# MaxHalford/sorobn

Measured on AMD Instinct MI355X. Metric: exact posterior queries/sec on 100-node 4-state grid BN, higher is better.
Workload: dtype f64

## Files before the change

__graft_entry__.py:

```python
import os
import subprocess
import sys

ROOT = os.path.dirname(os.path.abspath(__file__))
CSRC = os.path.join(ROOT, "sorobn_amd", "csrc")
LIB = os.path.join(ROOT, "sorobn_amd", "libmibn.so")
SOURCES = [os.path.join(CSRC, f) for f in ("planner.cpp", "engine.hip")]
DEPS = SOURCES + [os.path.join(CSRC, f) for f in ("planner.h", "plan_policy.h", "device_mem.h", "emit_core.h", "order_search.h", "ve_kernel.hip.h", "sweep_kernel.hip.h", "tiny_kernel.hip.h", "gibbs_kernel.hip.h", "sampler_plan.h",
                                              "sample_kernel.hip.h", "count_kernel.hip.h", "wave_prims.h", "wave_plan.h", "wave_plan_kernel.hip.h", "elim_kernel.hip.h", "draw_kernel.hip.h", "expect_kernel.hip.h", "score_kernel.hip.h", "citest_kernel.hip.h", "likelihood_kernel.hip.h", "bp_plan.h", "bp_kernel.hip.h", "count_weighted_kernel.hip.h")] + \
    [os.path.join(ROOT, "include", "mibn.h")]


def _stale(target, deps):
    if not os.path.exists(target):
        return True
    t = os.path.getmtime(target)
    return any(os.path.getmtime(d) > t for d in deps)


def build(force: bool = False) -> None:
    hipcc = os.environ.get("HIPCC", "/opt/rocm/bin/hipcc")
    if force or _stale(LIB, DEPS):
        cmd = [hipcc, "--offload-arch=gfx950", "-O3", "-mpopcnt", "-std=c++17", "-fPIC", "-shared",
               "-Wno-unused-value", "-Wno-unused-result", "-I", os.path.join(ROOT, "include"),
               "-o", LIB, *SOURCES, "-lpthread", "-ldl"]
        print("[build]", " ".join(cmd), flush=True)
        subprocess.check_call(cmd)
    subprocess.check_call(["make", "-C", os.path.join(ROOT, "oracle"), "-s"])
    if ROOT not in sys.path:
        sys.path.insert(0, ROOT)
    import sorobn_amd
    from sorobn_amd import _capi
    L = _capi.lib()
    missing = [s for s in _capi.SYMBOLS if not hasattr(L, s)]
    assert not missing, f"libmibn.so lacks {missing}"
    print("[build] ok:", L.mibn_version().decode(), flush=True)


def smoke() -> None:
    for p in (ROOT, os.path.join(ROOT, "tests")):
        if p not in sys.path:
            sys.path.insert(0, p)
    import numpy as np

    import netspec
    import sorobn_amd
    from oracle.oracle import OracleNet

    nets = netspec.load(os.path.join(ROOT, "tests", "golden", "examples.json"))
    alarm = next(n for n in nets if n["spec"]["name"] == "alarm")["spec"]
    checks = [(alarm, ("Burglary",), {"Mary calls": True, "John calls": True}),
              (netspec.grid_spec(4, 4, 4), ("000",), {"015": 0}),
              (netspec.grid_spec(6, 6, 4), ("035", "007"), {"000": 0, "020": 3})]
    for spec, q, ev in checks:
        bn = netspec.build(spec, sorobn_amd.BayesNet).use_device(0)
        ans = bn.query(*q, event=ev)
        names, labels, vals = OracleNet(spec).query(q, ev)
        assert list(ans.index.names) == names, (ans.index.names, names)
        assert [k if isinstance(k, tuple) else (k,) for k in ans.index.tolist()] == labels
        err = float(np.max(np.abs(ans.to_numpy() - vals)))
        assert err <= 1e-9, err
        print(f"[smoke] {spec['name']} P({', '.join(q)}) = {ans.to_numpy().tolist()} max|err| vs oracle {err:.2e}",
              flush=True)
    import golden_util as gu
    entry = gu.load("grid10x10.json")
    bn = netspec.build(gu.grid_spec_from_recipe(entry), sorobn_amd.BayesNet).use_device(0)
    reqs = [r for r in entry["requests"] if r["query"] == ["099"] and r["event"] == [["000", 0]]] + entry["requests"][:6]
    answers = bn.query_many([(tuple(r["query"]), {k: v for k, v in r["event"]}) for r in reqs])
    worst = 0.0
    for r, ans in zip(reqs, answers):
        name, inames, rows, vals, multi = gu.expected(r)
        assert ans.name == name and list(ans.index.names) == inames
        gu.assert_rows_equal(ans.index.tolist(), rows, ctx=str(r["query"]))
        worst = max(worst, float(np.max(np.abs(ans.to_numpy() - vals))))
    assert worst <= gu.TOL, worst
    st = bn.backend.engine.stats()
    print(f"[smoke] 10x10 K=4 grid: {len(reqs)} requests vs the reference's own answers, max|err| {worst:.2e}; "
          f"{st['alg_bytes'] / 1e6:.0f} MB algorithmic in {st['kernel_ms']:.2f} ms of kernels", flush=True)
    bn.backend.engine.set_option("second_on_device", 1)
    bn.backend.engine.set_option("gpu_emit", 2)
    again = bn.query_many([(tuple(r["query"]), {k: v for k, v in r["event"]}) for r in reqs])
    assert all(np.array_equal(a.to_numpy(), b.to_numpy()) for a, b in zip(answers, again))
    planned = [k for k in bn.backend.engine.kernel_stats() if k["name"] == "order_kernel+emit_kernel"]
    assert planned and planned[0]["items"] == len(reqs), planned
    print(f"[smoke] device planner: {len(reqs)} programs word for word the host's, posteriors bit for bit", flush=True)
    print("[smoke] ok", flush=True)


if __name__ == "__main__":
    build(force="--force" in sys.argv)
    if "--smoke" in sys.argv:
# ... 2 lines not shown
```

sorobn_amd/csrc/engine.hip:

```cpp
#include <hip/hip_runtime.h>
#include <dlfcn.h>
#include <rccl/rccl.h>

#include <algorithm>
#include <atomic>
#include <chrono>
#include <condition_variable>
#include <cstdio>
#include <cstdlib>
#include <cstring>
#include <limits>
#include <memory>
#include <mutex>
#include <numeric>
#include <string>
#include <thread>
#include <vector>

#include "../../include/mibn.h"
#include "device_mem.h"
#include "gibbs_kernel.hip.h"
#include "bp_kernel.hip.h"
#include "sample_kernel.hip.h"
#include "count_kernel.hip.h"
#include "count_weighted_kernel.hip.h"
#include "score_kernel.hip.h"
#include "citest_kernel.hip.h"
#include "planner.h"
#include "plan_policy.h"
#include "tiny_kernel.hip.h"
#include "sweep_kernel.hip.h"
#include "ve_kernel.hip.h"
#include "draw_kernel.hip.h"
#include "elim_kernel.hip.h"
#include "expect_kernel.hip.h"
#include "likelihood_kernel.hip.h"
#include "wave_plan_kernel.hip.h"

using namespace mibn;

namespace {
double now_ms() {
    return std::chrono::duration<double, std::milli>(std::chrono::steady_clock::now().time_since_epoch()).count();
}
}

struct OrderArgs {
    OrderNet net;
    const int64_t *q_off, *e_off;
    const int32_t *q_vars, *e_vars;
    int64_t B;
    uint32_t flags;
    uint8_t *orders;
    int32_t *order_len;
    OrderScratch *scratch;
    uint32_t *zero;
    const int32_t *perm;
    int32_t lanes;
};

#ifndef MIBN_ORDER_WAVES_PER_EU
#define MIBN_ORDER_WAVES_PER_EU 4
#endif
#ifndef MIBN_EMIT_WAVES_PER_EU
#define MIBN_EMIT_WAVES_PER_EU 4
#endif
#ifndef MIBN_PLAN_WG
#define MIBN_PLAN_WG 1024
#endif
__global__ __launch_bounds__(MIBN_PLAN_WG, MIBN_ORDER_WAVES_PER_EU) void order_kernel(const OrderArgs A) {
    if (A.zero && blockIdx.x == 0 && threadIdx.x == 0) *A.zero = 0;
    const int lane = (int)(threadIdx.x & 63), wave = (int)(threadIdx.x >> 6), waves = (int)(blockDim.x >> 6);
    if (lane >= A.lanes) return;
    const int64_t pos = ((int64_t)blockIdx.x * waves + wave) * A.lanes + lane;
    if (pos >= A.B) return;
    const int64_t b = A.perm ? A.perm[pos] : pos;
    OrderScratch &S = A.scratch[pos];
    const int64_t q0 = A.q_off[b], e0 = A.e_off[b];
    order_search(A.net, S, (int)(A.q_off[b + 1] - q0), A.q_vars + q0, (int)(A.e_off[b + 1] - e0), A.e_vars + e0,
                 (A.flags & MIBN_Q_NOPRUNE) != 0);
    uint8_t *out = A.orders + b * 128;
    for (int i = 0; i < S.n_best; ++i) out[i] = S.best[i];
    A.order_len[b] = S.n_best;
}

struct EmitArgs {
    EmitNet net;
    const int64_t *q_off, *e_off, *out_off;
    const int32_t *q_vars, *e_vars, *e_codes;
    const char *skip;
    const uint8_t *orders;
    const int32_t *order_len;
    int64_t B;
    uint32_t flags;
    uint32_t *prog;
    uint32_t prog_stride;
    EmitMeta *meta;
    Tag *tags;
    uint32_t *tag_cursor;
    uint32_t tag_cap;
    char *scratch;
    size_t scratch_stride;
    const int32_t *perm;
    int32_t lanes;
};

#if defined(MIBN_EMIT_PROF)
__device__ unsigned long long g_emit_prof[12];
#endif

__global__ __launch_bounds__(MIBN_PLAN_WG, MIBN_EMIT_WAVES_PER_EU) void emit_kernel(const EmitArgs A) {
    const int lane = (int)(threadIdx.x & 63), wave = (int)(threadIdx.x >> 6), waves = (int)(blockDim.x >> 6);
    if (lane >= A.lanes) return;
    const int64_t pos = ((int64_t)blockIdx.x * waves + wave) * A.lanes + lane;
    if (pos >= A.B) return;
    const int64_t b = A.perm ? A.perm[pos] : pos;
    EmitMeta m;
    m.words = 1; m.n_tags = 0; m.tag_first = 0; m.err = 0; m.prog_first = 0; m.pad_ = 0;
    m.alg_bytes = m.alg_flops = m.n_steps = m.max_step_cells = 0;
    m.arena_cells = 0;
    uint32_t *slot = A.prog + (size_t)b * A.prog_stride;
    if (A.skip[b]) { slot[0] = 0; A.meta[b] = m; return; }
// ... 175 lines not shown
    int set_cursor = 0;
    uint64_t call_id = 0;
    struct Comm {
        Stream stream;
        void *dl = nullptr;
        ncclComm_t comm = nullptr;
        int rank = 0, world = 1;
        decltype(&ncclGetUniqueId) GetUniqueId = nullptr;
        decltype(&ncclCommInitRank) CommInitRank = nullptr;
        decltype(&ncclCommDestroy) CommDestroy = nullptr;
        decltype(&ncclCommCount) CommCount = nullptr;
        decltype(&ncclCommUserRank) CommUserRank = nullptr;
        decltype(&ncclAllGather) AllGather = nullptr;
        decltype(&ncclReduce) Reduce = nullptr;
        decltype(&ncclAllReduce) AllReduce = nullptr;
        decltype(&ncclGetErrorString) GetErrorString = nullptr;
        DevBuf<char> d_send, d_recv;
    } comm;
    std::string err;
    mibn_stats stats{}, total{};
    mibn_kernel_stat kstats[kStatSlots];
    mibn_kernel_stat ktotal[kStatSlots];
    struct Elim {
        std::vector<ProgBuf> bufs;
        BatchPlan plan;
        Schedule sched;
        std::vector<LaunchGroup> groups;
        DevBuf<uint32_t> d_prog;
        DevBuf<uint64_t> d_prog_off, d_arena_off;
        DevBuf<Item> d_items;
        DevBuf<uint32_t> d_wg_item;
        DevBuf<double> d_m, d_log_p;
        DevBuf<int32_t> d_codes;
        DevBuf<DrawItem> d_draw_items;
        DevBuf<int64_t> d_m_off;
        ChunkSeeds seeds;
        std::vector<Event> ev;
        ~Elim() { for (ProgBuf &b : bufs) b.release(); }
    } elim;
    struct Expect {
        ExpectPlan plan;
        const double *weight = nullptr;
        int64_t B = 0, n_acc = 0;
        double *acc = nullptr, *p_out = nullptr;
        DevBuf<char> d_meta;
        DevBuf<double> d_f64;
        Event ev[2];
    } ex;
    bool expect = false;
    Findings staged;
    bool has_staged = false;
    const Findings *lh = nullptr;
    struct Dataset {
        DevBuf<uint8_t> d_codes;
        int64_t n_rows = 0;
        int32_t n_cols = 0;
        std::vector<int32_t> card;
        bool live = false;
        DevBuf<uint32_t> d_weights;
        int32_t n_sets = 0;
        std::vector<int64_t> weight_sum;
    };
    std::vector<Dataset> datasets;
    struct Score {
        DevBuf<unsigned long long> d_counts;
        DevBuf<char> d_meta;
        DevBuf<double> d_f64;
        DevBuf<long long> d_i64;
        std::vector<Event> ev;
    } sc;
    int64_t score_cells = kScoreCellBudget;
    int weighted_share = 1;
    double arena_gb = 200.0;
    int mfma_kernel = 1;
    int seg_kernel = 1;
    Event epoch;
    Event lane_ev, zero_ev;
    double busy_until = 0;
    int n_streams = 1;
    int first_chunk = 1;
    int threads = 0;
    int trace = 0;
    int split_kinds = 0;
    int overlap = 1;
    int sweep_dma = 1;
    int gibbs_lds = 1;
    int bp_lds = 1;
    int64_t chunk = 32768;
};

#define HIP_TRY(h, expr)                                                                              \
    do {                                                                                              \
        hipError_t e_ = (expr);                                                                       \
        if (e_ != hipSuccess) {                                                                       \
            (h)->err = std::string(#expr) + ": " + hipGetErrorString(e_);                             \
            return MIBN_E_HIP;                                                                        \
        }                                                                                             \
    } while (0)

static int upload_order_net(mibn_ctx *h) {
    h->order_net_ok = false;
    if (h->planner_only || h->net.n_vars > 128 || h->net.n_vars < 1) return MIBN_OK;
    const Network &net = h->net;
    const size_t n = (size_t)net.n_vars, nh = net.hint_sorted.size();
    std::vector<char> buf;
    auto put = [&](const void *p, size_t bytes) {
        const size_t off = (buf.size() + 15) & ~size_t(15);
        buf.resize(off + bytes);
        if (bytes) std::memcpy(buf.data() + off, p, bytes);
        return off;
    };
    const size_t o_card = put(net.card.data(), n * 4), o_depth = put(net.depth.data(), n * 4);
    const size_t o_asc = put(net.topo_asc.data(), n * 4), o_desc = put(net.topo_desc.data(), n * 4);
    const size_t o_hint = put(net.hint_flat.data(), nh * n * 4), o_log = put(net.log2card.data(), n * 8);
    const size_t o_anc = put(net.anc2.data(), n * sizeof(B2)), o_sc = put(net.scope2.data(), n * sizeof(B2));
    const size_t o_fam = put(net.fam2.data(), n * sizeof(B2));
    HIP_TRY(h, h->d_order_net.reset(buf.size()));
    HIP_TRY(h, hipMemcpy(h->d_order_net, buf.data(), buf.size(), hipMemcpyHostToDevice));
    OrderNet &o = h->order_net_dev;
    o = net.order_view();
    char *d = h->d_order_net;
    o.card = reinterpret_cast<const int32_t *>(d + o_card);
    o.depth = reinterpret_cast<const int32_t *>(d + o_depth);
    o.topo_asc = reinterpret_cast<const int32_t *>(d + o_asc);
    o.topo_desc = reinterpret_cast<const int32_t *>(d + o_desc);
    o.hint_sorted = reinterpret_cast<const int32_t *>(d + o_hint);
    o.log2card = reinterpret_cast<const double *>(d + o_log);
    o.anc = reinterpret_cast<const B2 *>(d + o_anc);
    o.cpt_scope = reinterpret_cast<const B2 *>(d + o_sc);
    o.fam = reinterpret_cast<const B2 *>(d + o_fam);
    h->order_net_ok = true;
    return MIBN_OK;
}

static int upload_emit_net(mibn_ctx *h) {
    h->emit_net_ok = false;
    if (h->planner_only || h->net.n_vars > 128 || h->net.n_vars < 1) return MIBN_OK;
    const Network &net = h->net;
    const size_t n = (size_t)net.n_vars;
    std::vector<char> buf;
    auto put = [&](const void *p, size_t bytes) {
        const size_t off = (buf.size() + 15) & ~size_t(15);
        buf.resize(off + bytes);
        if (bytes) std::memcpy(buf.data() + off, p, bytes);
        return off;
    };
    const size_t o_card = put(net.card.data(), n * 4), o_log = put(net.log2card.data(), n * 8), o_pool = put(net.pool_off.data(), n * 8);
    const size_t o_soff = put(net.scope_off32.data(), (n + 1) * 4), o_sv = put(net.scope_flat.data(), net.scope_flat.size() * 4);
    const size_t o_ss = put(net.cstride_flat.data(), net.cstride_flat.size() * 8), o_anc = put(net.anc_flat.data(), net.anc_flat.size() * 8);
    HIP_TRY(h, h->d_emit_net.reset(buf.size()));
    HIP_TRY(h, hipMemcpy(h->d_emit_net, buf.data(), buf.size(), hipMemcpyHostToDevice));
    EmitNet &e = h->emit_net_dev;
    e = net.emit_view();
    char *d = h->d_emit_net;
    e.card = reinterpret_cast<const int32_t *>(d + o_card);
    e.log2card = reinterpret_cast<const double *>(d + o_log);
    e.pool_off = reinterpret_cast<const int64_t *>(d + o_pool);
    e.scope_off = reinterpret_cast<const int32_t *>(d + o_soff);
    e.scope_vars = reinterpret_cast<const int32_t *>(d + o_sv);
    e.scope_stride = reinterpret_cast<const int64_t *>(d + o_ss);
    e.anc = reinterpret_cast<const uint64_t *>(d + o_anc);
    h->emit_net_ok = true;
    return MIBN_OK;
}

enum : unsigned { kNeedIdle = 1, kNeedDevice = 2, kNeedNet = 4 };
static int check_state(mibn_ctx *h, unsigned need) {
    if ((need & kNeedIdle) && (h->pend[0].active || h->pend[1].active)) { h->err = "asynchronous calls in flight: collect them with mibn_wait first"; return MIBN_E_STATE; }
    if ((need & kNeedDevice) && h->planner_only) { h->err = "planner-only context: no HIP device bound (there is no CPU fallback)"; return MIBN_E_NODEVICE; }
    if ((need & kNeedNet) && !h->has_net) { h->err = "set_network first"; return MIBN_E_STATE; }
    return MIBN_OK;
}

extern "C" {

const char *mibn_version(void) { return "mibn 0.1 (gfx950)"; }

int mibn_device_count(int *count) {
    int n = 0;
    if (hipGetDeviceCount(&n) != hipSuccess) n = 0;
    if (count) *count = n;
    return MIBN_OK;
}

constexpr int kEngineSmallCells = 512;

int mibn_create_planner(mibn_t **out) {
    if (!out) return MIBN_E_ARG;
    auto *h = new mibn_ctx();
    h->net.order_effort = 1; h->net.second_above = h->pol.base_second_above;
    h->net.small_cells = kEngineSmallCells;
    h->net.minfill_above = h->pol.base_minfill;
    h->planner_only = true;
    *out = h;
    return MIBN_OK;
}

int mibn_create(int device, mibn_t **out) {
    if (!out) return MIBN_E_ARG;
    *out = nullptr;
    int n = 0;
    if (hipGetDeviceCount(&n) != hipSuccess || n <= 0) return MIBN_E_NODEVICE;
    if (device < 0 || device >= n) return MIBN_E_ARG;
    auto *h = new mibn_ctx();
    h->net.order_effort = 1; h->net.second_above = h->pol.base_second_above;
    h->net.small_cells = kEngineSmallCells;
    h->net.minfill_above = h->pol.base_minfill;
    h->device = device;
    if (hipSetDevice(device) != hipSuccess) { delete h; return MIBN_E_NODEVICE; }
    hipDeviceProp_t prop;
    if (hipGetDeviceProperties(&prop, device) != hipSuccess) { delete h; return MIBN_E_NODEVICE; }
    if (std::string(prop.gcnArchName).rfind("gfx950", 0) != 0) {
        delete h;
        return MIBN_E_NODEVICE;
    }
    h->n_cu = prop.multiProcessorCount;
    bool ok = true;
    for (Stream *q : {&h->stream, &h->stream2, &h->aux[0][0], &h->aux[0][1], &h->aux[1][0], &h->aux[1][1], &h->aux[0][2], &h->aux[1][2], &h->copy_stream})
        ok = ok && q->ensure(hipStreamNonBlocking) == hipSuccess;
    ok = ok && hipFuncSetAttribute((const void *)ve_sweep_kernel, hipFuncAttributeMaxDynamicSharedMemorySize, kSweepLdsBytes) == hipSuccess;
    ok = ok && hipFuncSetAttribute((const void *)ve_sweep_dma_kernel, hipFuncAttributeMaxDynamicSharedMemorySize, kSweepLdsBytes) == hipSuccess;
    if (!ok) { delete h; return MIBN_E_HIP; }
    *out = h;
    return MIBN_OK;
}

void mibn_destroy(mibn_t *h) {
    if (!h) return;
    if (!h->planner_only) {
        (void)hipSetDevice(h->device);
        if (h->stream) (void)hipStreamSynchronize(h->stream);
        if (h->stream2) (void)hipStreamSynchronize(h->stream2);
        (void)mibn_comm_destroy(h);
    }
    delete h;
}

const char *mibn_last_error(const mibn_t *h) { return h ? h->err.c_str() : "null handle"; }

int mibn_set_option(mibn_t *h, const char *name, double value) {
    if (!h || !name) return MIBN_E_ARG;
    std::string n(name);
    if (n == "arena_gb") h->arena_gb = value;
    else if (n == "threads") h->threads = (int)value;
    else if (n == "chunk") h->chunk = std::max<int64_t>(1, (int64_t)value);
    else if (n == "big_iters") h->net.big_iters = std::max<int64_t>(1, (int64_t)value);
    else if (n == "tile_h") h->net.tile_h = std::max(0, std::min(kTileMax, (int)value));
    else if (n == "tile_kb") h->net.tile_bytes = std::max<int64_t>(16, (int64_t)value) << 10;
    else if (n == "chunk_sets") { if (mibn_drain(h) != MIBN_OK) return MIBN_E_HIP; h->n_sets = std::max(2, std::min(kChunkSets, (int)value)); h->set_cursor = 0; }
    else if (n == "trace") h->trace = (int)value;
    else if (n == "split_kinds") h->split_kinds = value != 0;
    else if (n == "overlap") { if (mibn_drain(h) != MIBN_OK) return MIBN_E_HIP; h->overlap = value != 0; }
    else if (n == "sweep_dma") h->sweep_dma = value != 0;
    else if (n == "seg_kernel") h->seg_kernel = value != 0;
    else if (n == "gibbs_lds") h->gibbs_lds = std::max(0, std::min(2, (int)value));
    else if (n == "bp_lds") h->bp_lds = value != 0;
    else if (n == "tiny") h->tiny = value != 0;
    else if (n == "tiny_zero_copy") h->tiny_zero_copy = value != 0;
    else if (n == "mfma_kernel") h->mfma_kernel = value != 0;
    else if (n == "gpu_emit") h->gpu_emit = std::max(0, std::min(2, (int)value));
    else if (n == "wave_wgs") h->wave_wgs = std::max(0, (int)value);
    else if (n == "plan_priority") h->plan_priority = std::max(0, std::min(2, (int)value));
    else if (n == "wave_plan") h->wave_plan = value != 0;
    else if (n == "plan_waves") h->plan_waves = std::max(1, std::min(16, (int)value));
    else if (n == "plan_sort") h->plan_sort = (int)value;
    else if (n == "wave_sort") h->wave_sort = value != 0;
    else if (n == "plan_lanes") h->plan_lanes = std::max(0, std::min(64, (int)value));
    else if (n == "emit_share") { h->pol.emit_share_opt = value > 0 ? std::min(1.0, value) : -1; if (value > 0) h->pol.emit_share = h->pol.emit_share_opt; }
    else if (n == "emit_words") h->emit_words = (uint32_t)std::max(1024, std::min(1 << 20, (int)value));
    else if (n == "gpu_search") h->gpu_search = std::max(0, std::min(2, (int)value));
    else if (n == "adaptive") {
        h->pol.adaptive = value != 0;
        if (!h->pol.adaptive) {
            h->net.minfill_above = h->pol.base_minfill;
            if (h->pol.auto_emit) { h->gpu_emit = 0; h->pol.auto_emit = false; }
            if (h->pol.auto_search) { h->gpu_search = 0; h->pol.auto_search = false; }
            h->pol.adaptive_seeded = false;
        }
    }
    else if (n == "minfill_above") { h->pol.base_minfill = value; h->net.minfill_above = value; }
    else if (n == "fuse") h->net.fuse = value != 0;
    else if (n == "plan_cache") h->net.plan_cache = value != 0;
    else if (n == "chain") h->net.chain = value != 0;
    else if (n == "streams") { if (mibn_drain(h) != MIBN_OK) return MIBN_E_HIP; h->n_streams = value >= 2 ? 2 : 1; h->n_sets = 2 * h->n_streams; h->set_cursor = 0; }
    else if (n == "first_chunk") h->first_chunk = std::max(0, std::min(2, (int)value));
    else if (n == "builtin_sweeps") {
        h->net.builtin_sweeps = value != 0;
        if (h->net.n_vars > 0) {
            std::vector<int32_t> flat;
            for (const auto &hh : h->net.hints) flat.insert(flat.end(), hh.begin(), hh.end());
            h->net.set_hints((int32_t)h->net.hints.size(), flat.data());
            if (!h->planner_only) return upload_order_net(h);
        }
    }
    else if (n == "order_effort") h->net.order_effort = std::max(0, std::min(1, (int)value));
    else if (n == "second_above") { h->pol.base_second_above = value; h->net.second_above = value; }
    else if (n == "second_on_device") h->second_on_device = value != 0;
    else if (n == "order_weights") h->net.order_weights = std::max(0, std::min(64, (int)value));
    else if (n == "sweep_canon") h->net.sweep_canon = value != 0;
    else if (n == "sweep_adapt") h->net.sweep_adapt = std::max(0, (int)value);
    else if (n == "sweep_min") h->net.sweep_min = std::max(2, std::min(5, (int)value));
    else if (n == "sweep_iters") h->net.sweep_iters = std::max(1, std::min(kTileMax, (int)value));
    else if (n == "sweep") h->net.sweep = std::max(0, std::min(5, (int)value));
    else if (n == "outer") h->net.outer = value != 0;
    else if (n == "stagger") h->net.stagger = std::max(1, std::min(8, (int)value));
    else if (n == "prune") h->net.prune = value != 0;
    else if (n == "weighted_share") h->weighted_share = value != 0;
    else if (n == "score_cells") h->score_cells = std::max<int64_t>(1, std::min<int64_t>(int64_t(1) << 28, (int64_t)value));
    else if (n == "small_cells") h->net.small_cells = std::max(1, std::min(kMaxT, (int)value));
    else { h->err = "unknown option " + n; return MIBN_E_ARG; }
    return MIBN_OK;
}

int mibn_set_network(mibn_t *h, int32_t n_vars, const int32_t *card, const int64_t *scope_off,
                     const int32_t *scope_vars, const int64_t *value_off, const double *values) {
    if (!h || !card || !scope_off || !scope_vars || !value_off || !values) return MIBN_E_ARG;
    std::string e = h->net.set(n_vars, card, scope_off, scope_vars, value_off, values);
    if (!e.empty()) { h->err = e; h->has_net = false; return MIBN_E_ARG; }
    h->has_net = true;
    h->pol.adaptive_seeded = false;
    if (h->pol.auto_emit) { h->gpu_emit = 0; h->pol.auto_emit = false; }
    if (!h->planner_only) {
        HIP_TRY(h, hipSetDevice(h->device));
        HIP_TRY(h, h->d_pool.reset(std::max<size_t>(1, h->net.pool.size())));
        HIP_TRY(h, hipMemcpy(h->d_pool, h->net.pool.data(), h->net.pool.size() * sizeof(double), hipMemcpyHostToDevice));
        h->tiny_ok = tiny_eligible(h->net);
        HIP_TRY(h, h->d_tiny_meta.release());
        if (h->tiny_ok) {
            const std::vector<int32_t> meta = tiny_meta(h->net);
            h->tiny_meta_words = (int32_t)meta.size();
            HIP_TRY(h, h->d_tiny_meta.reset(meta.size()));
            HIP_TRY(h, hipMemcpy(h->d_tiny_meta, meta.data(), meta.size() * 4, hipMemcpyHostToDevice));
            h->tiny_ok = tiny_lds_bytes((int)h->net.pool.size(), h->tiny_meta_words) <= 64 * 1024;
        }
// ... 258 lines not shown
    if ((rc = plan_stream(h))) return rc;
    const size_t nq = (size_t)(q_off[b1] - q_off[b0]), ne = (size_t)(e_off[b1] - e_off[b0]);
    const size_t off_bytes = (size_t)(n + 1) * 8;
    const size_t in_bytes = 2 * off_bytes + (nq + ne) * 4 + 64;
    if ((rc = pinned(h, h->search_in, in_bytes))) return rc;
    if ((rc = pinned(h, h->search_out, (size_t)n * 132))) return rc;
    if ((rc = ensure(h, h->d_order_scratch, (size_t)std::min(n, kSearchSlice)))) return rc;
    int64_t *qo = reinterpret_cast<int64_t *>(h->search_in.get()), *eo = qo + (n + 1);
    for (int64_t i = 0; i <= n; ++i) { qo[i] = q_off[b0 + i] - q_off[b0]; eo[i] = e_off[b0 + i] - e_off[b0]; }
    char *pv = h->search_in.get() + 2 * off_bytes;
    std::memcpy(pv, q_vars + q_off[b0], nq * 4);
    if (ne) std::memcpy(pv + nq * 4, e_vars + e_off[b0], ne * 4);
    const char *d_req = h->search_in.get();
    uint8_t *orders_out = reinterpret_cast<uint8_t *>(h->search_out.get());
    int32_t *len_out = reinterpret_cast<int32_t *>(h->search_out.get() + (size_t)n * 128);
    for (int64_t s0 = 0; s0 < n; s0 += kSearchSlice) {
        const int64_t m = std::min(kSearchSlice, n - s0);
        OrderArgs A;
        A.net = h->order_net_dev;
        A.net.prune = h->net.prune;
        A.net.minfill_above = h->net.minfill_above;
        {
            const OrderNet hv = h->net.order_view();
            A.net.chain_weight = hv.chain_weight;
            A.net.big_cells = hv.big_cells;
            A.net.effort = hv.effort;
        }
        A.q_off = reinterpret_cast<const int64_t *>(d_req) + s0;
        A.e_off = reinterpret_cast<const int64_t *>(d_req + off_bytes) + s0;
        A.q_vars = reinterpret_cast<const int32_t *>(d_req + 2 * off_bytes);
        A.e_vars = A.q_vars + nq;
        A.B = m;
        A.flags = flags;
        A.orders = orders_out + s0 * 128;
        A.order_len = len_out + s0;
        A.scratch = h->d_order_scratch;
        A.zero = nullptr;
        A.perm = nullptr;
        A.lanes = plan_lanes_now(h);
        {
            const int64_t per_wg = (int64_t)A.lanes * h->plan_waves;
            hipLaunchKernelGGL(order_kernel, dim3((unsigned)((m + per_wg - 1) / per_wg)), dim3(64 * h->plan_waves), 0, h->search_stream, A);
        }
        HIP_TRY(h, hipGetLastError());
    }
    return MIBN_OK;
}

int search_wait(mibn_ctx *h) {
    HIP_TRY(h, hipStreamSynchronize(h->search_stream));
    return MIBN_OK;
}

constexpr int64_t kPlanSlice = 32768;
int plan_on_device_launch(mibn_ctx *h, uint32_t flags, int64_t b0, int64_t b1, const int64_t *q_off, const int32_t *q_vars, const int64_t *e_off,
                          const int32_t *e_vars, const int32_t *e_codes, const int64_t *out_off, const char *skip, mibn_ctx::Set &st, size_t prog_words) {
    const int64_t n = b1 - b0;
    int rc;
    if ((rc = plan_stream(h))) return rc;
    hipStream_t P = h->search_stream;
    const size_t nq = (size_t)(q_off[b1] - q_off[b0]), ne = (size_t)(e_off[b1] - e_off[b0]);
    const size_t off_bytes = (size_t)(n + 1) * 8;
    const size_t perm_off = (3 * off_bytes + (nq + 2 * ne) * 4 + (size_t)n + 63) & ~(size_t)63;
    const size_t in_bytes = perm_off + (size_t)n * 4 + 64;
    const size_t stride = h->emit_words;
    const size_t tag_cap = (size_t)n * 64;
    const size_t scratch_stride = emit_scratch_bytes(h->net.n_vars);
    const int64_t slice = std::min(n, kPlanSlice);
    bool wave = false;
    if (h->wave_plan && h->order_net_ok) {
        if (!h->wnet_host) { h->wnet_host.reset(new WNet); std::memset(h->wnet_host.get(), 0, sizeof(WNet)); h->wnet_ok = false; }
        std::unique_ptr<WNet> fresh(new WNet);
        if (h->net.wave_view(*fresh)) {
            if (!h->d_wnet) HIP_TRY(h, h->d_wnet.reset(1));
            if (!h->wnet_ok || std::memcmp(fresh.get(), h->wnet_host.get(), sizeof(WNet)) != 0) {
                HIP_TRY(h, hipMemcpy(h->d_wnet, fresh.get(), sizeof(WNet), hipMemcpyHostToDevice));
                std::memcpy(h->wnet_host.get(), fresh.get(), sizeof(WNet));
                h->wnet_ok = true;
            }
            wave = true;
        }
    }
    if ((rc = pinned(h, h->emit_in, in_bytes))) return rc;
    if ((rc = pinned(h, h->emit_out, (size_t)n * sizeof(EmitMeta) + tag_cap * sizeof(Tag) + 64))) return rc;
    if (!h->d_emit_cursor) HIP_TRY(h, h->d_emit_cursor.reset(16));
    if (!wave) {
    if ((rc = ensure(h, h->d_orders, (size_t)n * 128))) return rc;
    if ((rc = ensure(h, h->d_order_len, (size_t)n))) return rc;
    if ((rc = ensure(h, h->d_order_scratch, (size_t)slice))) return rc;
    }
    if (!wave && (size_t)slice * scratch_stride > h->d_emit_scratch.cap())
        HIP_TRY(h, h->d_emit_scratch.reset((size_t)std::max<int64_t>(slice, std::min<int64_t>(h->chunk, kPlanSlice)) * scratch_stride));
    if ((rc = ensure(h, st.d_prog, std::max(prog_words, (size_t)n * stride) + kMaxStepWords))) return rc;
    HIP_TRY(h, h->emit_ev[0].ensure());
    HIP_TRY(h, h->emit_ev[1].ensure());
    char *pin = h->emit_in.get();
    int64_t *qo = reinterpret_cast<int64_t *>(pin), *eo = qo + (n + 1), *oo = eo + (n + 1);
    for (int64_t i = 0; i <= n; ++i) { qo[i] = q_off[b0 + i] - q_off[b0]; eo[i] = e_off[b0 + i] - e_off[b0]; oo[i] = out_off[b0 + i] - out_off[b0]; }
    char *pv = pin + 3 * off_bytes;
    std::memcpy(pv, q_vars + q_off[b0], nq * 4);
    if (ne) { std::memcpy(pv + nq * 4, e_vars + e_off[b0], ne * 4); std::memcpy(pv + (nq + ne) * 4, e_codes + e_off[b0], ne * 4); }
    std::memcpy(pv + (nq + 2 * ne) * 4, skip + b0, (size_t)n);
    int32_t *perm = reinterpret_cast<int32_t *>(pin + perm_off);
    const bool sorted = h->plan_sort && h->net.n_vars <= 128 && !h->net.anc2.empty();
    if (sorted) {
        std::vector<uint8_t> key((size_t)std::min(n, kPlanSlice));
        for (int64_t s0 = 0; s0 < n; s0 += kPlanSlice) {
            const int64_t m = std::min(kPlanSlice, n - s0);
            int32_t count[130] = {0};
            for (int64_t i = 0; i < m; ++i) {
                const int64_t b = b0 + s0 + i;
                B2 rel;
                for (int64_t k = q_off[b]; k < q_off[b + 1]; ++k) { const int v = q_vars[k]; rel.set(v); rel.a |= h->net.anc2[v].a; rel.b |= h->net.anc2[v].b; }
                for (int64_t k = e_off[b]; k < e_off[b + 1]; ++k) { const int v = e_vars[k]; rel.set(v); rel.a |= h->net.anc2[v].a; rel.b |= h->net.anc2[v].b; }
                const int c = 128 - b2_count(rel);
                key[(size_t)i] = (uint8_t)c;
                ++count[c + 1];
            }
            for (int c = 0; c < 129; ++c) count[c + 1] += count[c];
            if (h->plan_sort == 1) {
                for (int64_t i = 0; i < m; ++i) perm[s0 + count[key[(size_t)i]]++] = (int32_t)i;
            } else {
                const int64_t per = h->plan_sort == 3 ? (int64_t)plan_lanes_now(h) : (int64_t)plan_lanes_now(h) * h->plan_waves, G = (m + per - 1) / per;
                std::vector<int32_t> rank_of((size_t)m);
                for (int64_t i = 0; i < m; ++i) rank_of[(size_t)count[key[(size_t)i]]++] = (int32_t)i;
                std::vector<int64_t> fill((size_t)G, 0);
                int64_t g = 0;
                for (int64_t r = 0; r < m; ++r) {
                    for (int tries = 0; tries < G; ++tries, g = (g + 1) % G) {
                        const int64_t pos = g * per + fill[(size_t)g];
                        if (fill[(size_t)g] < per && pos < m) { perm[s0 + pos] = rank_of[(size_t)r]; ++fill[(size_t)g]; g = (g + 1) % G; break; }
                    }
                }
            }
        }
    }
    HIP_TRY(h, hipEventRecord(h->emit_ev[0], P));
    const char *d = pin;
    EmitMeta *meta_out = reinterpret_cast<EmitMeta *>(h->emit_out.get());
    Tag *tags_out = reinterpret_cast<Tag *>(h->emit_out.get() + (size_t)n * sizeof(EmitMeta) + 64);
    if (wave) {
        WavePlanArgs A;
        A.net = h->d_wnet;
        A.anc = h->order_net_dev.anc;
        A.q_off = reinterpret_cast<const int64_t *>(d);
        A.e_off = reinterpret_cast<const int64_t *>(d + off_bytes);
        A.out_off = reinterpret_cast<const int64_t *>(d + 2 * off_bytes);
        A.q_vars = reinterpret_cast<const int32_t *>(d + 3 * off_bytes);
        A.e_vars = A.q_vars + nq;
        A.e_codes = A.e_vars + ne;
        A.skip = reinterpret_cast<const char *>(A.e_codes + ne);
        A.B = n;
        A.flags = flags;
        A.prog = st.d_prog;
        A.prog_stride = (uint32_t)stride;
        A.meta = meta_out;
        A.tags = tags_out;
        A.tag_cursor = h->d_emit_cursor;
        A.tag_cap = (uint32_t)tag_cap;
        A.perm = nullptr;
        if (h->wave_sort && n > 4 * kWaveWG * (int64_t)h->n_cu) {
            if ((rc = ensure(h, h->d_plan_perm, 2 * (size_t)n))) return rc;
            A.perm = h->d_plan_perm;
        }
        hipLaunchKernelGGL(reset_cursor_kernel, dim3(1), dim3(1), 0, P, h->d_emit_cursor);
        if (A.perm) hipLaunchKernelGGL(plan_sort_kernel, dim3(1), dim3(kPlanSortThreads), 0, P, A);
        {
            int64_t grid = std::min<int64_t>((n + kWaveWG - 1) / kWaveWG, (int64_t)h->n_cu * MIBN_WAVE_MIN_WGS);
            if (h->wave_wgs > 0) grid = std::min<int64_t>(grid, h->wave_wgs);
            hipLaunchKernelGGL(wave_plan_kernel, dim3((unsigned)grid), dim3(64 * kWaveWG), 0, P, A);
        }
        HIP_TRY(h, hipGetLastError());
    }
    for (int64_t s0 = 0; !wave && s0 < n; s0 += kPlanSlice) {
        const int64_t m = std::min(kPlanSlice, n - s0);
        OrderArgs O;
        O.net = h->order_net_dev;
        O.net.prune = h->net.prune;
        O.net.minfill_above = h->net.minfill_above;
        {
            const OrderNet hv = h->net.order_view();
            O.net.chain_weight = hv.chain_weight;
            O.net.big_cells = hv.big_cells;
            O.net.effort = hv.effort;
        }
        O.q_off = reinterpret_cast<const int64_t *>(d) + s0;
        O.e_off = reinterpret_cast<const int64_t *>(d + off_bytes) + s0;
        O.q_vars = reinterpret_cast<const int32_t *>(d + 3 * off_bytes);
        O.e_vars = O.q_vars + nq;
        O.B = m;
        O.flags = flags;
        O.orders = h->d_orders + s0 * 128;
        O.order_len = h->d_order_len + s0;
        O.scratch = h->d_order_scratch;
        O.zero = s0 == 0 ? h->d_emit_cursor : nullptr;
        O.perm = sorted ? reinterpret_cast<const int32_t *>(d + perm_off) + s0 : nullptr;
        O.lanes = plan_lanes_now(h);
        const int64_t per_wg = (int64_t)O.lanes * h->plan_waves;
        hipLaunchKernelGGL(order_kernel, dim3((unsigned)((m + per_wg - 1) / per_wg)), dim3(64 * h->plan_waves), 0, P, O);
        EmitArgs A;
        {
            A.net = h->net.emit_view();
            const EmitNet &dv = h->emit_net_dev;
            A.net.card = dv.card; A.net.log2card = dv.log2card; A.net.pool_off = dv.pool_off; A.net.scope_off = dv.scope_off;
            A.net.scope_vars = dv.scope_vars; A.net.scope_stride = dv.scope_stride; A.net.anc = dv.anc;
        }
        A.q_off = O.q_off;
        A.e_off = O.e_off;
        A.out_off = reinterpret_cast<const int64_t *>(d + 2 * off_bytes) + s0;
        A.q_vars = O.q_vars;
        A.e_vars = O.e_vars;
        A.e_codes = A.e_vars + ne;
        A.skip = reinterpret_cast<const char *>(A.e_codes + ne) + s0;
        A.orders = O.orders;
        A.order_len = O.order_len;
        A.B = m;
        A.flags = flags;
        A.prog = st.d_prog + (size_t)s0 * stride;
        A.prog_stride = (uint32_t)stride;
        A.meta = meta_out + s0;
        A.tags = tags_out;
        A.tag_cursor = h->d_emit_cursor;
        A.tag_cap = (uint32_t)tag_cap;
        A.scratch = h->d_emit_scratch;
        A.scratch_stride = scratch_stride;
        A.perm = O.perm;
        A.lanes = plan_lanes_now(h);
        hipLaunchKernelGGL(emit_kernel, dim3((unsigned)((m + per_wg - 1) / per_wg)), dim3(64 * h->plan_waves), 0, P, A);
        HIP_TRY(h, hipGetLastError());
    }
    HIP_TRY(h, hipEventRecord(h->emit_ev[1], P));
    return MIBN_OK;
}

int plan_on_device_collect(mibn_ctx *h, int64_t b0, int64_t n, BatchPlan &ck, double *dev_ms, std::vector<int64_t> *beyond_list) {
    hipStream_t P = h->search_stream;
    const size_t stride = h->emit_words;
    const size_t tag_cap = (size_t)n * 64;
    const EmitMeta *meta = reinterpret_cast<const EmitMeta *>(h->emit_out.get());
    const Tag *tags = reinterpret_cast<const Tag *>(h->emit_out.get() + (size_t)n * sizeof(EmitMeta) + 64);
    HIP_TRY(h, hipStreamSynchronize(P));
    {
        float ms = 0;
        HIP_TRY(h, hipEventElapsedTime(&ms, h->emit_ev[0], h->emit_ev[1]));
        if (dev_ms) *dev_ms = ms;
    }
    size_t n_tags = 0;
    for (int64_t i = 0; i < n; ++i)
        if (!meta[i].err) n_tags = std::max<size_t>(n_tags, (size_t)meta[i].tag_first + meta[i].n_tags);
    n_tags = std::min(n_tags, tag_cap);
    ck.st = PlanStats{};
    ck.arena_cells = 0;
    ck.err.clear();
    ck.prog_off.assign(n, 0);
    ck.cost.assign(n, 0.0);
    ck.arena_need.assign(n, 0);
    ck.thread_of.assign(n, 0);
    ck.local_off.assign(n, 0);
    ck.thread_words.clear();
    ck.tag_first.assign(n, 0);
    ck.tag_count.assign(n, 0);
    ck.tags.resize(1);
    ck.tags[0].assign(tags, tags + n_tags);
    bool refused = false, beyond = false;
    for (int64_t i = 0; i < n; ++i) {
        const EmitMeta &m = meta[i];
        if (m.err == kEmitErrWords) { refused = true; continue; }
        if (m.err == kEmitErrDevice) {
            if (beyond_list && beyond_list->size() < 256) { beyond_list->push_back(i); continue; }
            refused = true; beyond = true; continue;
        }
        if (m.err) { h->err = "request " + std::to_string(b0 + i) + ": " + emit_error_message(m.err); return MIBN_E_LIMIT; }
        ck.prog_off[i] = (uint64_t)i * stride + m.prog_first;
        ck.local_off[i] = ck.prog_off[i];
        ck.tag_first[i] = m.tag_first;
        ck.tag_count[i] = m.n_tags;
        ck.cost[i] = m.alg_bytes;
        ck.arena_need[i] = m.arena_cells;
        ck.st.alg_bytes += m.alg_bytes;
        ck.st.alg_flops += m.alg_flops;
        ck.st.n_steps += m.n_steps;
        ck.st.max_step_cells = std::max(ck.st.max_step_cells, m.max_step_cells);
        ck.arena_cells = std::max(ck.arena_cells, m.arena_cells);
    }
    ck.total_words = (size_t)n * stride;
    if (refused) {
        if (h->trace || h->emit_fallbacks < 4) {
            int64_t nw = 0, nb = 0, first = -1;
            for (int64_t i = 0; i < n; ++i) { nw += meta[i].err == kEmitErrWords; nb += meta[i].err == kEmitErrDevice; if (meta[i].err && first < 0) first = i; }
            std::fprintf(stderr, "[mibn plan] device planner: %lld requests beyond a device limit, %lld did not fit their slot / the item buffer (first: request %lld, %u words, %u items; %zu items of %zu in the buffer): the host plans the chunk\n",
                         (long long)nb, (long long)nw, (long long)(b0 + first), first >= 0 ? meta[first].words : 0u, first >= 0 ? meta[first].n_tags : 0u, n_tags, tag_cap);
        }
        if (!beyond) h->emit_words = std::min<uint32_t>(h->emit_words * 2, 1u << 20);
        ++h->emit_fallbacks;
        return 1;
    }
    ++h->emit_chunks;
    return MIBN_OK;
}

constexpr int64_t kTinyZeroCopyRequests = 64;

int expect_run(mibn_t *h, const double *d_results) {
    mibn_ctx::Expect &X = h->ex;
    const ExpectPlan &P = X.plan;
    int rc;
    std::vector<char> meta;
    auto put = [&](const void *src, size_t bytes) {
        const size_t o = meta.size();
        meta.resize(o + ((bytes + 7) & ~size_t(7)));
        if (bytes) std::memcpy(meta.data() + o, src, bytes);
        return o;
    };
    const size_t o_req = put(P.req.data(), P.req.size() * sizeof(ExpectReq)), o_big = put(P.big.data(), P.big.size() * sizeof(ExpectReq));
    const size_t o_ds = put(P.dim_stride.data(), P.dim_stride.size() * 8), o_sl = put(P.slab_lo.data(), P.slab_lo.size() * 8);
    const size_t o_sp = put(P.slab_part.data(), P.slab_part.size() * 8), o_dc = put(P.dim_card.data(), P.dim_card.size() * 4);
    const size_t o_sb = put(P.slab_begin.data(), P.slab_begin.size() * 4), o_sc = put(P.slab_cells.data(), P.slab_cells.size() * 4);
    const size_t o_bb = put(P.blk_begin.data(), P.blk_begin.size() * 4), o_bs = put(P.blk_slab.data(), P.blk_slab.size() * 4);
    if ((rc = ensure(h, X.d_meta, meta.size() + 16))) return rc;
    const size_t nB = (size_t)X.B, nA = (size_t)X.n_acc;
    const size_t f_acc = 0, f_p = nA, f_w = f_p + nB, f_part = f_w + (X.weight ? nB : 0);
    if ((rc = ensure(h, X.d_f64, f_part + (size_t)P.part_cells + 2))) return rc;
    for (Event &e : X.ev) HIP_TRY(h, e.ensure());
    const hipStream_t S = h->stream;
    HIP_TRY(h, hipMemcpyAsync(X.d_meta, meta.data(), meta.size(), hipMemcpyHostToDevice, S));
    if (nA) HIP_TRY(h, hipMemcpyAsync(X.d_f64 + f_acc, X.acc, nA * 8, hipMemcpyHostToDevice, S));
    if (X.weight) HIP_TRY(h, hipMemcpyAsync(X.d_f64 + f_w, X.weight, nB * 8, hipMemcpyHostToDevice, S));
    HIP_TRY(h, hipMemsetAsync(X.d_f64 + f_p, 0, nB * 8, S));
    const size_t n_slabs = P.slab_cells.size();
    double launches = 0;
    HIP_TRY(h, hipEventRecord(X.ev[0], S));
    if (n_slabs) {
        ExpectArgs A;
        A.results = d_results;
        A.req = reinterpret_cast<const ExpectReq *>(X.d_meta + o_req);
        A.dim_card = reinterpret_cast<const int32_t *>(X.d_meta + o_dc);
        A.dim_stride = reinterpret_cast<const int64_t *>(X.d_meta + o_ds);
        A.weight = X.weight ? X.d_f64 + f_w : nullptr;
        A.slab_begin = reinterpret_cast<const int32_t *>(X.d_meta + o_sb);
        A.slab_cells = reinterpret_cast<const int32_t *>(X.d_meta + o_sc);
        A.slab_part = reinterpret_cast<const int64_t *>(X.d_meta + o_sp);
        A.part = X.d_f64 + f_part;
        A.p_out = X.d_f64 + f_p;
        hipLaunchKernelGGL(expect_kernel, dim3((unsigned)n_slabs), dim3(64), 0, S, A);
        launches += 1;
    }
// ... 285 lines not shown
        if (R.out_off[b + 1] - R.out_off[b] != cells) { h->err = "request " + std::to_string(b) + ": out_off does not match the query table size"; return MIBN_E_ARG; }
        if (evidence_outside_domain(h->net, rq, R.e_codes + R.e_off[b])) R.skip[(size_t)b] = 1;
        if (R.raw && rq.nq == 0 && rq.ne == 0 && rq.nl == 0 && h->net.prune && !(R.flags & MIBN_Q_NOPRUNE)) R.skip[(size_t)b] = 2;
    }
    return MIBN_OK;
}

int query_setup(QueryRun &R) {
    mibn_ctx *h = R.h;
    int rc;
    R.res_cells = (size_t)(R.out_off[R.B] - R.out_off[0]);
    if ((rc = ensure(h, h->d_results[R.slot], R.res_cells))) return rc;
    R.d_results = h->d_results[R.slot];
    R.n_lanes = h->n_streams > 1 ? 2 : 1;
    {
        bool idle = true;
        for (auto &st : h->set) idle = idle && !st.busy;
        if (!h->epoch) { HIP_TRY(h, h->epoch.ensure()); idle = true; }
        if (idle) {
            HIP_TRY(h, hipEventRecord(h->epoch, h->stream));
            h->busy_until = 0;
        }
    }
    HIP_TRY(h, hipMemsetAsync(R.d_results, 0, R.res_cells * 8, h->stream));
    if (R.n_lanes > 1) {
        HIP_TRY(h, h->zero_ev.ensure(hipEventDisableTiming));
        HIP_TRY(h, hipEventRecord(h->zero_ev, h->stream));
        HIP_TRY(h, hipStreamWaitEvent(h->stream2, h->zero_ev, 0));
    }
    size_t free_b = 0, total_b = 0;
    HIP_TRY(h, hipMemGetInfo(&free_b, &total_b));
    R.budget_cells = (int64_t)(std::min(h->arena_gb * 1e9, 0.8 * (double)(free_b + h->d_arena[0].cap() + h->d_arena[1].cap())) / 8.0) / R.n_lanes;
    bool effort_ok = true;
    if (h->net.order_effort >= 1 && (h->gpu_emit || h->gpu_search) && !R.host_only) {
        std::unique_ptr<WNet> probe(new WNet);
        effort_ok = h->wave_plan && h->net.wave_view(*probe);
    }
    R.emit_on = !R.host_only && h->gpu_emit && h->order_net_ok && h->emit_net_ok && effort_ok;
    h->net.second_above = (R.emit_on && !h->second_on_device) ? 1e300 : h->pol.base_second_above;
    R.search_on = !R.host_only && !R.emit_on && h->gpu_search && h->order_net_ok && h->net.order_effort < 1;
    for (auto &st : h->set) R.gpu_busy = R.gpu_busy || (st.busy && st.ev_used && hipEventQuery(st.ev[st.ev_used - 1]) == hipErrorNotReady);
    (void)hipGetLastError();
    R.short_first = h->first_chunk == 2 || (h->first_chunk == 1 && !R.gpu_busy);
    return MIBN_OK;
}

int64_t chunk_size(const QueryRun &R, int64_t b0) {
    const mibn_ctx *h = R.h;
    if (b0 == 0 && R.search_on && h->gpu_search == 1) return std::max<int64_t>(1024, h->chunk / 8);
    if (R.emit_on) return h->chunk;
    if (b0 == 0 && R.short_first && (R.B > h->chunk || !R.gpu_busy)) return std::max<int64_t>(1024, h->chunk / 4);
    return h->chunk;
}

int search_window(QueryRun &R, int64_t b0, int64_t b1, double t0, const uint8_t *&orders, const int32_t *&order_len) {
    mibn_ctx *h = R.h;
    int rc;
    if (h->gpu_search == 2) {
        if ((rc = search_orders_async(h, R.flags, b0, b1, R.q_off, R.q_vars, R.e_off, R.e_vars))) return rc;
        if ((rc = search_wait(h))) return rc;
        orders = reinterpret_cast<const uint8_t *>(h->search_out.get());
        order_len = reinterpret_cast<const int32_t *>(h->search_out.get() + (size_t)(b1 - b0) * 128);
    } else if (R.n_chunks == 0 && b1 < R.B) {
        if ((rc = search_orders_async(h, R.flags, b1, R.B, R.q_off, R.q_vars, R.e_off, R.e_vars))) return rc;
        R.search_b0 = b1;
    } else if (R.search_b0 >= 0) {
        if (!R.search_done) { if ((rc = search_wait(h))) return rc; R.search_done = true; h->search_ms += now_ms() - t0; }
        orders = reinterpret_cast<const uint8_t *>(h->search_out.get()) + (size_t)(b0 - R.search_b0) * 128;
        order_len = reinterpret_cast<const int32_t *>(h->search_out.get() + (size_t)(R.B - R.search_b0) * 128) + (b0 - R.search_b0);
    }
    return MIBN_OK;
}

size_t join_plans(BatchPlan &ck, BatchPlan &dp, BatchPlan &hp, int64_t nd, size_t stride) {
    const int T = (int)hp.tags.size();
    ck.st = dp.st;
    ck.st.alg_bytes += hp.st.alg_bytes; ck.st.alg_flops += hp.st.alg_flops; ck.st.n_steps += hp.st.n_steps;
    ck.st.max_step_cells = std::max(dp.st.max_step_cells, hp.st.max_step_cells);
    ck.arena_cells = std::max(dp.arena_cells, hp.arena_cells);
    ck.err.clear();
    ck.tags.resize((size_t)T + 1);
    for (int t = 0; t < T; ++t) ck.tags[(size_t)t].swap(hp.tags[(size_t)t]);
    ck.tags[(size_t)T].swap(dp.tags[0]);
    ck.thread_words = hp.thread_words;
    auto join = [&](auto &dst, const auto &a, const auto &b) { dst.assign(a.begin(), a.end()); dst.insert(dst.end(), b.begin(), b.end()); };
    join(ck.cost, dp.cost, hp.cost);
    join(ck.arena_need, dp.arena_need, hp.arena_need);
    join(ck.tag_first, dp.tag_first, hp.tag_first);
    join(ck.tag_count, dp.tag_count, hp.tag_count);
    join(ck.local_off, dp.local_off, hp.local_off);
    ck.thread_of.assign((size_t)nd, T);
    ck.thread_of.insert(ck.thread_of.end(), hp.thread_of.begin(), hp.thread_of.end());
    const size_t prog_base = (size_t)nd * stride;
    ck.prog_off = dp.prog_off;
    for (uint64_t o : hp.prog_off) ck.prog_off.push_back(prog_base + o);
    ck.total_words = prog_base + hp.total_words;
    return prog_base;
}

int replan_beyond(QueryRun &R, mibn_ctx::Set &st, int64_t b0, int64_t nd, const std::vector<int64_t> &beyond, bool &on_device) {
    mibn_ctx *h = R.h;
    BatchPlan &ck = st.plan, &xp = st.xplan;
    std::vector<char> mask(R.skip.begin(), R.skip.end());
    for (int64_t i = 0; i < nd; ++i) mask[(size_t)(b0 + i)] = 1;
    for (int64_t i : beyond) mask[(size_t)(b0 + i)] = R.skip[(size_t)(b0 + i)];
    plan_batch(h->net, *h->pool, st.xbufs, b0, b0 + nd, R.q_off, R.q_vars, R.e_off, R.e_vars, R.e_codes, R.out_off, mask.data(), xp,
               (R.flags & MIBN_Q_NOPRUNE) != 0, nullptr, nullptr, b0);
    if (!xp.err.empty()) { h->err = xp.err; return MIBN_E_LIMIT; }
    const size_t stride = h->emit_words;
    const size_t X = ck.tags.size();
    ck.tags.resize(X + xp.tags.size());
    for (size_t t = 0; t < xp.tags.size(); ++t) ck.tags[X + t] = xp.tags[t];
    bool fits = true;
    for (int64_t i : beyond) {
        const uint32_t *w = st.xbufs[(size_t)xp.thread_of[(size_t)i]].data + xp.local_off[(size_t)i];
        size_t words = 1;
        for (uint32_t k = 0; k < w[0]; ++k) words += w[words + 6];
        if (words + kMaxStepWords > stride) { fits = false; break; }
        HIP_TRY(h, hipMemcpyAsync(st.d_prog + (size_t)i * stride, w, words * 4, hipMemcpyHostToDevice, h->copy_stream));
        ck.prog_off[(size_t)i] = (uint64_t)i * stride;
        ck.local_off[(size_t)i] = ck.prog_off[(size_t)i];
        ck.thread_of[(size_t)i] = (int32_t)(X + (size_t)xp.thread_of[(size_t)i]);
        ck.tag_first[(size_t)i] = xp.tag_first[(size_t)i];
        ck.tag_count[(size_t)i] = xp.tag_count[(size_t)i];
        ck.cost[(size_t)i] = xp.cost[(size_t)i];
        ck.arena_need[(size_t)i] = xp.arena_need[(size_t)i];
    }
    ck.st.alg_bytes += xp.st.alg_bytes; ck.st.alg_flops += xp.st.alg_flops; ck.st.n_steps += xp.st.n_steps;
    ck.st.max_step_cells = std::max(ck.st.max_step_cells, xp.st.max_step_cells);
    ck.arena_cells = std::max(ck.arena_cells, xp.arena_cells);
    if (h->trace || h->emit_single < 4)
        std::fprintf(stderr, "[mibn plan] device planner: %zu of %lld requests beyond a device limit (first: request %lld): planned on the host\n", beyond.size(), (long long)nd,
                     (long long)(b0 + beyond[0]));
    h->emit_single += (int64_t)beyond.size();
    if (!fits) on_device = false;
    return MIBN_OK;
}

int check_against_host(QueryRun &R, mibn_ctx::Set &st, int64_t b0, int64_t b1) {
    mibn_ctx *h = R.h;
    const BatchPlan &ck = st.plan;
    const int64_t n = b1 - b0;
    const size_t stride = h->emit_words;
    std::vector<uint32_t> dev((size_t)n * stride);
    HIP_TRY(h, hipStreamSynchronize(h->copy_stream));
    HIP_TRY(h, hipMemcpy(dev.data(), st.d_prog, dev.size() * 4, hipMemcpyDeviceToHost));
    BatchPlan ref;
    plan_batch(h->net, *h->pool, st.bufs, b0, b1, R.q_off, R.q_vars, R.e_off, R.e_vars, R.e_codes, R.out_off, R.skip.data(), ref,
               (R.flags & MIBN_Q_NOPRUNE) != 0, nullptr, nullptr);
    if (!ref.err.empty()) { h->err = ref.err; return MIBN_E_LIMIT; }
    for (int64_t i = 0; i < n; ++i) {
        const uint32_t *hw = st.bufs[ref.thread_of[i]].data + ref.local_off[i], *dw = dev.data() + (size_t)ck.prog_off[(size_t)i];
        size_t words = 1;
        for (uint32_t k = 0; k < hw[0]; ++k) words += hw[words + 6];
        for (size_t k = 0; k < words; ++k)
            if (hw[k] != dw[k]) {
                size_t off = 1, step = 0;
                while (step + 1 < hw[0] && off + hw[off + 6] <= k) { off += hw[off + 6]; ++step; }
                h->err = "device planner: request " + std::to_string(b0 + i) + " word " + std::to_string(k) + " of " + std::to_string(words) + " (step " + std::to_string(step) + " of " +
                         std::to_string(hw[0]) + ", kind " + std::to_string(hw[off] & 0xff) + ", word " + std::to_string(k - off) + " of the step's " + std::to_string(hw[off + 6]) + "): host " +
                         std::to_string(hw[k]) + " device " + std::to_string(dw[k]) + "; device program " + std::to_string(dw[0]) + " steps";
                return MIBN_E_STATE;
            }
        const Tag *ht = ref.tags[ref.thread_of[i]].data() + ref.tag_first[i], *dt = ck.tags[(size_t)ck.thread_of[i]].data() + ck.tag_first[i];
        bool same = ref.tag_count[i] == ck.tag_count[i] && ref.arena_need[i] == ck.arena_need[i] && ref.cost[i] == ck.cost[i];
        for (uint32_t k = 0; same && k < ref.tag_count[i]; ++k)
            same = ht[k].rel_off == dt[k].rel_off && ht[k].a == dt[k].a && ht[k].wgs == dt[k].wgs && ht[k].level == dt[k].level &&
                   ht[k].kid == dt[k].kid && ht[k].bytes == dt[k].bytes;
        if (!same) { h->err = "device planner: work items / statistics of request " + std::to_string(b0 + i) + " differ from the host's"; return MIBN_E_STATE; }
    }
    return MIBN_OK;
}

int plan_chunk(QueryRun &R, mibn_ctx::Set &st, int64_t b0, int64_t b1, bool &on_device, size_t &prog_base) {
    mibn_ctx *h = R.h;
    const int64_t n = b1 - b0;
    const bool no_prune = (R.flags & MIBN_Q_NOPRUNE) != 0;
    int rc;
    const double t0 = now_ms();
    const uint8_t *orders = nullptr;
    const int32_t *order_len = nullptr;
    if (R.search_on && (rc = search_window(R, b0, b1, t0, orders, order_len))) return rc;
    BatchPlan &ck = st.plan;
    on_device = false;
    prog_base = 0;
    std::vector<int64_t> beyond;
    int64_t nd = 0;
    if (R.emit_on) {
        nd = h->pol.device_share(n, h->gpu_emit == 2, wave_mode(h));
        const size_t stride = h->emit_words;
        if ((rc = plan_on_device_launch(h, R.flags, b0, b0 + nd, R.q_off, R.q_vars, R.e_off, R.e_vars, R.e_codes, R.out_off, R.skip.data(), st, (size_t)n * stride))) return rc;
        const double t_launched = now_ms();
        BatchPlan &hp = h->emit_host, &dp = h->emit_dev;
        double host_ms = 0, dev_ms = 0;
        if (nd < n) {
            const double th = now_ms();
            plan_batch(h->net, *h->pool, st.bufs, b0 + nd, b1, R.q_off, R.q_vars, R.e_off, R.e_vars, R.e_codes, R.out_off, R.skip.data(), hp, no_prune, nullptr, nullptr, b0);
            host_ms = now_ms() - th;
            R.call_plan_ms += host_ms;
            if (!hp.err.empty()) { h->err = hp.err; return MIBN_E_LIMIT; }
        }
        const double tw = now_ms();
        rc = plan_on_device_collect(h, b0, nd, nd < n ? dp : ck, &dev_ms, &beyond);
        h->emit_ms += now_ms() - tw;
        R.call_plan_ms += now_ms() - tw;
        if (h->trace >= 2) std::fprintf(stderr, "[mibn plan] collect returned %d at %.2f ms of the block\n", rc, now_ms() - t0);
        book_stat(h, kStatPlanner, 2, dev_ms, 0.0, (double)nd, true, true);
// ... 33 lines not shown
    h->stats.plan_ms += now_ms() - t0;
    if (h->trace >= 2) std::fprintf(stderr, "[mibn plan] chunk planning block %.2f ms (on the device: %d)\n", now_ms() - t0, (int)on_device);
    return MIBN_OK;
}

int upload_chunk(QueryRun &R, mibn_ctx::Set &st, int64_t b0, int64_t n, bool on_device, size_t prog_base) {
    mibn_ctx *h = R.h;
    const BatchPlan &ck = st.plan;
    int rc;
    if (!on_device && (rc = ensure(h, st.d_prog, ck.total_words + kMaxStepWords))) return rc;
    if ((rc = ensure(h, st.d_prog_off, (size_t)n))) return rc;
    if ((rc = ensure(h, st.d_arena_off, (size_t)n))) return rc;
    const double t0 = now_ms();
    if ((rc = upload_programs(h, st.d_prog, prog_base, st.bufs, ck, h->copy_stream))) return rc;
    if ((rc = upload(h, st.stage[0], st.d_prog_off, ck.prog_off.data(), (size_t)n * 8))) return rc;
    if (h->lh && (rc = upload_chunk_seeds(h, st.seeds, ck, b0, n, R.skip.data(), h->copy_stream))) return rc;
    h->stats.h2d_ms += now_ms() - t0;
    return MIBN_OK;
}

struct LevelKernel { void (*kernel)(LevelArgs); unsigned block, lds_bytes; int stream, slot; };
constexpr LevelKernel kLevelKernels[kNumLevelRoutes] = {
     {ve_level_kernel, kWG, 0, 0, kStatLevel},
     {ve_sweep_dma_kernel, kSweepWG, kSweepLdsBytes, 1, kStatSweepDma},
     {ve_sweep_kernel, kSweepWG, kSweepLdsBytes, 1, kKidSweep},
     {ve_segment_kernel, kWG, 0, 2, kStatSegment},
     {ve_mfma_kernel, kWG, 0, 3, kStatMfma},
};
static_assert((int)LevelRoute::Level == 0 && (int)LevelRoute::SweepDma == 1 && (int)LevelRoute::SweepReg == 2 && (int)LevelRoute::Segment == 3 && (int)LevelRoute::Mfma == 4, "the rows' order");

struct LevelStreams {
    using Timed = mibn_ctx::Set::Timed;
    static constexpr int kNS = kLevelStreams;
    mibn_ctx *h;
    mibn_ctx::Set &st;
    const bool two;
    hipStream_t SS[kNS];
    long last[kNS], prev[kNS], saw[kNS][kNS];
    int cur_level = -1;
    Timed pair;

    LevelStreams(mibn_ctx *h_, mibn_ctx::Set &st_, int lane, hipStream_t S)
        : h(h_), st(st_), two(h_->overlap != 0), SS{S, h_->aux[lane][0], h_->aux[lane][1], h_->aux[lane][2]}, pair(fresh()) {
        for (int a = 0; a < kNS; ++a) { last[a] = prev[a] = -1; for (int b = 0; b < kNS; ++b) saw[a][b] = -1; }
    }
    Timed fresh() const { return Timed{Timed::kLevelGroup, Timed::kNone, Timed::kNone, 0.0, 0.0, h->call_id}; }
    void close_pair() {
        if (std::any_of(std::begin(pair.e), std::end(pair.e), [](const size_t (&p)[2]) { return p[0] != Timed::kNone; })) st.timed.push_back(pair);
        pair = fresh();
    }
    int begin(size_t e_first) {
        for (int j = 1; two && j < kNS; ++j) HIP_TRY(h, hipStreamWaitEvent(SS[j], st.ev[e_first], 0));
        return MIBN_OK;
    }
    int before(int level, int si) {
        if (!two) return MIBN_OK;
        if (level != cur_level) { cur_level = level; for (int j = 0; j < kNS; ++j) prev[j] = last[j]; close_pair(); }
        for (int j = 0; j < kNS; ++j)
            if (j != si && prev[j] > saw[si][j]) { HIP_TRY(h, hipStreamWaitEvent(SS[si], st.ev[(size_t)prev[j]], 0)); saw[si][j] = prev[j]; }
        return MIBN_OK;
    }
    void after(int si, size_t e0, size_t e1, double bytes, double grid) {
        if (!two) return;
        last[si] = (long)e1;
        if (h->split_kinds) return;
        pair.e[si][0] = e0; pair.e[si][1] = e1;
        pair.bytes += bytes;
        pair.items += grid;
    }
    int end() {
        if (!two) return MIBN_OK;
        close_pair();
        for (int j = 1; j < kNS; ++j)
            if (last[j] > saw[0][j]) HIP_TRY(h, hipStreamWaitEvent(SS[0], st.ev[(size_t)last[j]], 0));
        return MIBN_OK;
    }
};

int run_wave(QueryRun &R, mibn_ctx::Set &st, int lane, hipStream_t S, int64_t b0, int64_t r0, int64_t r1) {
    mibn_ctx *h = R.h;
    int rc;
    double t0 = now_ms();
    Schedule &sc = st.sched;
    build_schedule(h->net, st.plan, st.bufs, r0, r1, sc);
    h->stats.plan_ms += now_ms() - t0;
    R.call_fixed_ms += now_ms() - t0;
    if (h->trace) std::fprintf(stderr, "[mibn plan] build_schedule %.2f ms (%zu items, %zu workgroups, %zu launches)\n", now_ms() - t0, sc.items.size(), sc.wg_item.size(), sc.launches.size());
    const size_t need_bytes = (size_t)std::max<int64_t>(16, sc.arena_cells) * sizeof(double);
    if ((rc = grow_arena(h, lane, need_bytes, R.budget_cells, S))) return rc;
    if (r0 > 0) { HIP_TRY(h, hipStreamSynchronize(S)); HIP_TRY(h, hipStreamSynchronize(h->copy_stream)); }
    if ((rc = ensure(h, st.d_items, sc.items.size()))) return rc;
    if ((rc = ensure(h, st.d_wg_item, sc.wg_item.size()))) return rc;
    t0 = now_ms();
    if ((rc = upload(h, st.stage[1], st.d_arena_off, sc.arena_off.data(), (size_t)(r1 - r0) * 8))) return rc;
    if ((rc = upload(h, st.stage[2], st.d_items, sc.items.data(), sc.items.size() * sizeof(Item)))) return rc;
    if ((rc = upload(h, st.stage[3], st.d_wg_item, sc.wg_item.data(), sc.wg_item.size() * sizeof(uint32_t)))) return rc;
    HIP_TRY(h, st.uploaded.ensure(hipEventDisableTiming));
    HIP_TRY(h, hipEventRecord(st.uploaded, h->copy_stream));
    HIP_TRY(h, hipStreamWaitEvent(S, st.uploaded, 0));
    h->stats.h2d_ms += now_ms() - t0;
    LevelArgs A;
    A.prog = st.d_prog;
    A.prog_off = st.d_prog_off + r0;
    A.arena_off = st.d_arena_off;
    A.pool = h->d_pool;
    A.arena = h->arena(lane);
    A.results = R.d_results + (R.out_off[b0] - R.out_off[0]);
    A.items = st.d_items;
    double n_wg = 0;
    if (h->trace) st.gap_from = h->n_waves ? (int)((h->n_waves - 1) & 3) : -1;
    size_t e_first = 0, e_last = 0;
    if ((rc = next_event(h, st, e_first, S))) return rc;
    size_t e_begin = e_first;
    {
        SeedArgs SA;
        unsigned sgrid = 0;
        double sbytes = 0;
        if (wave_seeds(h, st.seeds, r0, r1, A.arena, st.d_arena_off, SA, sgrid, sbytes)) {
            size_t e0 = 0;
            if ((rc = next_event(h, st, e0, S))) return rc;
            hipLaunchKernelGGL(likelihood_seed_kernel, dim3(sgrid), dim3(kSeedWG), 0, S, SA);
            if ((rc = next_event(h, st, e_begin, S))) return rc;
            st.timed.push_back({kStatSeed, e0, e_begin, sbytes, (double)sgrid, h->call_id});
            n_wg += (double)sgrid;
        }
    }
    LevelStreams LS(h, st, lane, S);
    if ((rc = LS.begin(e_begin))) return rc;
    level_groups(sc, {h->split_kinds != 0, h->seg_kernel != 0, h->mfma_kernel != 0, h->sweep_dma != 0}, st.groups);
    for (const LaunchGroup &g : st.groups) {
        const LevelKernel &K = kLevelKernels[(int)g.route];
        A.wg_item = st.d_wg_item + g.wg_level;
        A.wg_base = (uint32_t)(g.wg_first - g.wg_level);
        size_t e0 = 0, e1 = 0;
        const int si = LS.two ? K.stream : 0;
        hipStream_t Sx = LS.SS[si];
        if ((rc = LS.before(g.level, si))) return rc;
        if ((rc = next_event(h, st, e0, Sx))) return rc;
        hipLaunchKernelGGL(K.kernel, dim3((unsigned)g.grid), dim3(K.block), K.lds_bytes, Sx, A);
        if ((rc = next_event(h, st, e1, Sx))) return rc;
        LS.after(si, e0, e1, g.alg_bytes, (double)g.grid);
        st.timed.push_back({g.stat_kid >= 0 && g.route != LevelRoute::SweepDma ? g.stat_kid : K.slot, e0, e1, g.alg_bytes, (double)g.grid, h->call_id});
        n_wg += (double)g.grid;
    }
    if ((rc = LS.end())) return rc;
    if ((rc = next_event(h, st, e_last, S))) return rc;
    st.timed.push_back({mibn_ctx::Set::Timed::kWave, e_first, e_last, 0.0, (double)(r1 - r0), h->call_id});
    HIP_TRY(h, hipGetLastError());
    if (h->trace) {
        Event &ge = h->gap_ev[h->n_waves & 3];
        HIP_TRY(h, ge.ensure());
        HIP_TRY(h, hipEventRecord(ge, S));
    }
    ++h->n_waves;
    st.busy = true;
    h->stats.arena_bytes = std::max(h->stats.arena_bytes, (double)need_bytes);
    h->stats.n_workgroups += n_wg;
    return MIBN_OK;
}

void fold_stats(mibn_ctx *h) {
    h->total.plan_ms += h->stats.plan_ms;
    h->total.h2d_ms += h->stats.h2d_ms;
    h->total.d2h_ms += h->stats.d2h_ms;
    h->total.total_ms += h->stats.total_ms;
    h->total.alg_bytes += h->stats.alg_bytes;
    h->total.alg_flops += h->stats.alg_flops;
// ... 1916 lines not shown
```

sorobn_amd/csrc/planner.cpp:

```cpp
#include "planner.h"

#include <algorithm>
#include <unordered_map>
#include <atomic>
#include <cmath>
#include <cstdlib>
#include <cstring>
#include <functional>
#include <limits>
#include <memory>
#include <numeric>
#include <condition_variable>
#include <mutex>
#include <thread>

namespace mibn {

#ifdef MIBN_PLAN_PROFILE
#include <chrono>
double g_prof[8];
struct ProfT { int k; std::chrono::steady_clock::time_point t0; ProfT(int k_) : k(k_), t0(std::chrono::steady_clock::now()) {} ~ProfT() { g_prof[k] += std::chrono::duration<double, std::micro>(std::chrono::steady_clock::now() - t0).count(); } };
#define PROF(k) ProfT prof_##k(k)
#else
#define PROF(k)
// ... 1116 lines not shown
    std::vector<uint32_t> finals;
    std::vector<Tag> tags;
    PlanStats st;
};

struct TemplateStore {
    struct Shard {
        std::mutex m;
        std::unordered_map<std::string, std::unique_ptr<PlanTemplate>> map;
    };
    static constexpr int kShards = 64;
    static constexpr size_t kMaxWords = 64u << 20;
    Shard shard[kShards];
    std::atomic<size_t> words{0};
    uint64_t version = 0, opt_sig = 0;
    void clear() {
        for (auto &sh : shard) sh.map.clear();
        words = 0;
    }
};

struct PlanCache {
    const TemplateStore *store = nullptr;
    uint64_t version = 0;
    uint64_t seen = 0, probe_hits = 0;
    bool on = true;
    static constexpr uint64_t kMinWindow = 1024, kMaxWindow = 65536, kProbe = 256;
    uint64_t window = kMinWindow;
    PlanRecord rec;
    std::string key;
};

uint64_t option_signature(const Network &net) {
    uint64_t h = 1469598103934665603ull;
    auto mix = [&](uint64_t v) { h = (h ^ v) * 1099511628211ull; };
    mix((uint64_t)net.small_cells); mix((uint64_t)net.big_iters); mix((uint64_t)net.tile_h); mix((uint64_t)net.fuse);
    mix((uint64_t)net.chain); mix((uint64_t)net.sweep); mix((uint64_t)net.sweep_iters); mix((uint64_t)net.sweep_min); mix((uint64_t)net.sweep_adapt); mix((uint64_t)net.order_weights); mix((uint64_t)net.order_effort); mix((uint64_t)net.second_above); mix((uint64_t)net.hint_sorted.size()); mix((uint64_t)net.sweep_canon); mix((uint64_t)net.outer); mix((uint64_t)net.prune); mix((uint64_t)net.minfill_above);
    mix((uint64_t)net.hints.size()); mix((uint64_t)net.tile_bytes);
    return h;
}

TemplateStore *template_store(const Network &net) {
    if (!net.templates) net.templates = std::make_shared<TemplateStore>();
    TemplateStore *ts = static_cast<TemplateStore *>(net.templates.get());
    const uint64_t sig = option_signature(net);
    if (ts->version != net.version || ts->opt_sig != sig || ts->words.load() > TemplateStore::kMaxWords) {
        ts->clear();
        ts->version = net.version;
        ts->opt_sig = sig;
    }
    return ts;
}

PlanCache &plan_cache(const TemplateStore *ts) {
    static thread_local PlanCache c;
    if (c.store != ts || c.version != ts->version) {
        c.store = ts;
        c.version = ts->version;
        c.seen = c.probe_hits = 0;
        c.on = true;
        c.window = PlanCache::kMinWindow;
    }
    return c;
}

}

void plan_batch(const Network &net, ThreadPool &pool, std::vector<ProgBuf> &bufs, int64_t b0, int64_t b1,
                const int64_t *q_off, const int32_t *q_vars, const int64_t *e_off, const int32_t *e_vars,
                const int32_t *e_codes, const int64_t *out_off, const char *skip, BatchPlan &ck, bool no_prune,
                const uint8_t *orders, const int32_t *order_len, int64_t out_first, ProgramKind kind, const int64_t *l_off,
                const int32_t *l_vars) {
    const int64_t n = b1 - b0;
    const int T = pool.size();
    if ((int)bufs.size() < T) bufs.resize(T);
    ck.st = PlanStats{};
    ck.arena_cells = 0;
    ck.err.clear();
    ck.prog_off.assign(n, 0);
    ck.cost.assign(n, 0.0);
    ck.arena_need.assign(n, 0);
    ck.thread_of.assign(n, 0);
    ck.local_off.assign(n, 0);
    ck.thread_words.assign(T, 0);
    ck.tag_first.assign(n, 0);
    ck.tag_count.assign(n, 0);
    if ((int)ck.tags.size() < T) ck.tags.resize(T);
    std::vector<PlanStats> tst(T);
    std::vector<std::string> terr(T);
    TemplateStore *store = (net.plan_cache && may_use_templates(kind) && !l_off) ? template_store(net) : nullptr;
    std::atomic<int64_t> next{0};
    constexpr int64_t kBlock = 32;
    const EmitNet en = net.emit_view();
    pool.run([&](int t) {
        ProgBuf &prog = bufs[t];
        prog.size = 0;
        std::vector<Tag> &tags = ck.tags[t];
        tags.clear();
        for (;;) {
          const int64_t lo = next.fetch_add(kBlock, std::memory_order_relaxed);
          if (lo >= n) break;
          const int64_t hi = std::min(n, lo + kBlock);
          for (int64_t i = lo; i < hi; ++i) {
            const int64_t b = b0 + i;
            ck.prog_off[i] = prog.size;
            ck.local_off[i] = prog.size;
            ck.thread_of[i] = t;
            ck.tag_first[i] = (uint32_t)tags.size();
            if (skip && skip[b]) {
                put_empty_program(prog, kind, (int32_t)(e_off[b + 1] - e_off[b]), e_vars + e_off[b], e_codes + e_off[b]);
                continue;
            }
            Request rq;
            rq.nq = (int32_t)(q_off[b + 1] - q_off[b]);
            rq.qvars = q_vars + q_off[b];
            rq.ne = (int32_t)(e_off[b + 1] - e_off[b]);
            rq.evars = e_vars + e_off[b];
            rq.ecodes = e_codes + e_off[b];
            rq.out_off = out_off[b] - out_off[out_first >= 0 ? out_first : b0];
            rq.no_prune = no_prune;
            rq.kind = kind;
            if (orders) { rq.order = orders + (size_t)i * 128; rq.n_order = order_len[i]; }
            if (l_off) { rq.nl = (int32_t)(l_off[b + 1] - l_off[b]); rq.lvars = l_vars + l_off[b]; }
            PlanStats st;
            PlanCache *pc = store ? &plan_cache(store) : nullptr;
            bool use_cache = false;
            if (pc) {
                const uint64_t w = pc->seen++;
                if (w == 0) { pc->probe_hits = 0; pc->on = true; }
                if (w == PlanCache::kProbe) {
                    pc->on = pc->probe_hits * 4 >= PlanCache::kProbe;
                    pc->window = pc->on ? PlanCache::kMinWindow : std::min(pc->window * 2, PlanCache::kMaxWindow);
                }
                if (pc->seen >= pc->window) pc->seen = 0;
                use_cache = pc->on;
            }
            if (use_cache) {
                std::string &key = pc->key;
                key.assign(reinterpret_cast<const char *>(&rq.nq), sizeof(rq.nq));
                key.push_back(no_prune ? 'N' : 'P');
                key.append(reinterpret_cast<const char *>(rq.qvars), sizeof(int32_t) * (size_t)rq.nq);
                key.append(reinterpret_cast<const char *>(rq.evars), sizeof(int32_t) * (size_t)rq.ne);
                TemplateStore::Shard &sh = store->shard[std::hash<std::string>{}(key) % TemplateStore::kShards];
                const PlanTemplate *hit = nullptr;
                {
                    std::lock_guard<std::mutex> lk(sh.m);
                    auto it = sh.map.find(key);
                    if (it != sh.map.end()) hit = it->second.get();
                }
                if (hit) {
                    const PlanTemplate &tp = *hit;
                    ++pc->probe_hits;
                    uint32_t *w = prog.extend(tp.words.size());
                    std::copy(tp.words.begin(), tp.words.end(), w);
                    for (const auto &pt : tp.patches) {
                        uint64_t off = pt.base;
                        for (uint32_t k = pt.first; k < pt.first + pt.count; ++k) off += (uint64_t)(tp.stride[k] * rq.ecodes[tp.slot[k]]);
                        off |= kConstFlag;
                        w[pt.pos] = (uint32_t)(off & 0xffffffffu);
                        w[pt.pos + 1] = (uint32_t)(off >> 32);
                    }
                    for (uint32_t fp : tp.finals) {
                        w[fp] = (uint32_t)((uint64_t)rq.out_off & 0xffffffffu);
                        w[fp + 1] = (uint32_t)((uint64_t)rq.out_off >> 32);
                    }
                    st = tp.st;
// ... 36 lines not shown
            tst[t].alg_bytes += st.alg_bytes;
            tst[t].alg_flops += st.alg_flops;
            tst[t].n_steps += st.n_steps;
            tst[t].max_step_cells = std::max(tst[t].max_step_cells, st.max_step_cells);
            tst[t].arena_cells = std::max(tst[t].arena_cells, st.arena_cells);
          }
        }
        ck.thread_words[t] = prog.size;
    });
    std::vector<size_t> tbase(T, 0);
    size_t base = 0;
    for (int t = 0; t < T; ++t) {
        tbase[t] = base;
        base += ck.thread_words[t];
    }
    for (int64_t i = 0; i < n; ++i) ck.prog_off[i] = tbase[ck.thread_of[i]] + ck.local_off[i];
    for (int t = 0; t < T; ++t) {
        if (!terr[t].empty()) ck.err = terr[t];
        ck.st.alg_bytes += tst[t].alg_bytes;
        ck.st.alg_flops += tst[t].alg_flops;
        ck.st.n_steps += tst[t].n_steps;
        ck.st.max_step_cells = std::max(ck.st.max_step_cells, tst[t].max_step_cells);
        ck.arena_cells = std::max(ck.arena_cells, tst[t].arena_cells);
    }
    ck.total_words = base;
}


const char *kernel_name(int kid) {
    static std::string names[kNumKernels];
    static bool init = false;
    if (!init) {
        names[kKidSeg] = "segments";
        static const char *cxn[3] = {"cx4", "cx16", "cxN"}, *ncn[6] = {"nc1", "nc4", "nc16", "ncN", "nc16-mfma", "outer-mfma"};
        for (int nb = 1; nb <= 2; ++nb)
            for (int c = 0; c < 3; ++c)
                for (int n = 0; n < 6; ++n)
                    names[kKidFiber0 + (nb - 1) * 18 + c * 6 + n] =
                        "fiber<" + std::to_string(nb) + "," + cxn[c] + "," + ncn[n] + ">";
        names[kKidChain] = "fiber<1,cx64,chain-mfma>";
        for (int j = 0; j < kMaxIn; ++j) names[kKidGeneric0 + j] = "generic<" + std::to_string(j + 1) + ">";
        names[kKidSweep] = "ve_sweep_kernel";
        init = true;
    }
    return kid >= 0 && kid < kNumKernels ? names[kid].c_str() : "?";
}

struct ClassOrder {
    int rank_of[kNumKernels] = {}, kid_at[kNumKernels] = {};
    constexpr ClassOrder() {
        int n = 0;
        bool seen[kNumKernels] = {};
        auto add = [&](int kid) { if (!seen[kid]) { seen[kid] = true; kid_at[n] = kid; rank_of[kid] = n++; } };
        add(kKidSeg);
        for (int j = 0; j < kMaxIn; ++j) add(kKidGeneric0 + j);
        constexpr int two_table_nc[4] = {3, 1, 2, 0};
        for (int n2 : two_table_nc)
            for (int c = 2; c >= 0; --c) add(kKidFiber0 + 18 + c * 6 + n2);
        for (int c = 2; c >= 0; --c) add(kKidFiber0 + c * 6 + 3);
        for (int k = 0; k < 6; ++k) add(kKidFiber0 + 2 * 6 + k);
        for (int c = 0; c < 2; ++c) add(kKidFiber0 + 18 + c * 6 + 5);
        for (int kid = 0; kid < kNumKernels; ++kid)
            if (!is_mfma1_class(kid) && kid != kKidSweep) add(kid);
        add(kKidMfma1Cx4);
        add(kKidMfma1Cx16);
        add(kKidSweep);
    }
    constexpr bool routes_contiguous() const {
        for (int k = 0; k < 16; ++k) {
            const LevelRouteOpts o{(k & 1) != 0, (k & 2) != 0, (k & 4) != 0, (k & 8) != 0};
            bool closed[kNumLevelRoutes] = {};
            for (int r = 0; r < kNumKernels; ++r) {
                const int route = (int)route_of(kid_at[r], o);
                if (closed[route]) return false;
                if (r + 1 < kNumKernels && (int)route_of(kid_at[r + 1], o) != route) closed[route] = true;
            }
        }
        return true;
    }
};
constexpr ClassOrder kClassOrder;
static_assert(kClassOrder.routes_contiguous(), "the classes of a kernel must be contiguous in the class order: level_groups merges neighbours only");

void build_schedule(const Network &net, const BatchPlan &bp, const std::vector<ProgBuf> &bufs, int64_t r0, int64_t r1,
                    Schedule &out) {
    (void)bufs;
    const int64_t n = r1 - r0;
    out.items.clear();
    out.wg_item.clear();
    out.launches.clear();
    out.arena_off.assign(n, 0);
    int64_t top = 0;
    for (int64_t i = 0; i < n; ++i) {
        out.arena_off[i] = (uint64_t)top;
        top += (bp.arena_need[r0 + i] + 15) & ~int64_t(15);
    }
    out.arena_cells = top;
    int n_levels = 0;
    size_t n_tags = 0, n_wg = 0;
    for (int64_t i = 0; i < n; ++i) {
        const int64_t r = r0 + i;
        const Tag *tg = bp.tags[bp.thread_of[r]].data() + bp.tag_first[r];
        const uint32_t cnt = bp.tag_count[r];
        if (cnt) n_levels = std::max(n_levels, (int)tg[cnt - 1].level + 1);
        n_tags += cnt;
    }
    const int G = std::max(1, std::min(net.stagger, 8));
    const int delta = G > 1 ? (n_levels + G - 1) / G : 0;
    auto shift = [&](int64_t i) { return (int)(i % G) * delta; };
    n_levels += (G - 1) * delta;
    out.n_levels = n_levels;
    const size_t nb = (size_t)n_levels * kNumKernels;
    std::vector<size_t> count(nb + 1, 0);
    std::vector<double> bytes(nb, 0.0);
    std::vector<uint64_t> sweep_tiles((size_t)n_levels, 0);
    for (int64_t i = 0; i < n; ++i) {
        const int64_t r = r0 + i;
        const Tag *tg = bp.tags[bp.thread_of[r]].data() + bp.tag_first[r];
        const int sh = shift(i);
        for (uint32_t k = 0; k < bp.tag_count[r]; ++k) {
            const size_t bkt = (size_t)(tg[k].level + sh) * kNumKernels + kClassOrder.rank_of[tg[k].kid];
            ++count[bkt + 1];
            bytes[bkt] += tg[k].bytes;
            if (tg[k].kid == kKidSweep) sweep_tiles[(size_t)(tg[k].level + sh)] += tg[k].a;
            else n_wg += tg[k].wgs;
        }
    }
    std::vector<uint32_t> sweep_iters((size_t)n_levels, (uint32_t)std::max(1, net.sweep_iters));
    if (net.sweep_adapt)
        for (int l = 0; l < n_levels; ++l)
            while (sweep_iters[(size_t)l] > 2 && sweep_tiles[(size_t)l] / sweep_iters[(size_t)l] < (uint64_t)net.sweep_adapt) sweep_iters[(size_t)l] /= 2;
    for (int64_t i = 0; i < n; ++i) {
        const int64_t r = r0 + i;
        const Tag *tg = bp.tags[bp.thread_of[r]].data() + bp.tag_first[r];
        const int sh = shift(i);
        for (uint32_t k = 0; k < bp.tag_count[r]; ++k)
            if (tg[k].kid == kKidSweep) { const uint32_t it = sweep_iters[(size_t)(tg[k].level + sh)]; n_wg += (tg[k].a + it - 1) / it; }
    }
    for (size_t k = 0; k < nb; ++k) count[k + 1] += count[k];
    out.items.resize(n_tags);
    std::vector<size_t> cur(count.begin(), count.end() - 1);
    for (int64_t i = 0; i < n; ++i) {
        const int64_t r = r0 + i;
        const Tag *tg = bp.tags[bp.thread_of[r]].data() + bp.tag_first[r];
        const int sh = shift(i);
        for (uint32_t k = 0; k < bp.tag_count[r]; ++k) {
            uint32_t a = tg[k].a, wgs = tg[k].wgs;
            if (tg[k].kid == kKidSweep) { const uint32_t it = sweep_iters[(size_t)(tg[k].level + sh)]; wgs = (a + it - 1) / it; a = it; }
            out.items[cur[(size_t)(tg[k].level + sh) * kNumKernels + kClassOrder.rank_of[tg[k].kid]]++] = Item{(uint32_t)i, tg[k].rel_off, a, wgs};
        }
    }
    out.wg_item.resize(n_wg);
    size_t wg = 0, wg_level = 0;
    int cur_level = -1;
    for (size_t k = 0; k < nb; ++k)
        if (count[k + 1] > count[k]) {
            const int level = (int)(k / kNumKernels), kid = kClassOrder.kid_at[k % kNumKernels];
            if (level != cur_level) { cur_level = level; wg_level = wg; }
            if (kid == kKidSeg && count[k + 1] - count[k] > 1) {
                Item *first = out.items.data() + count[k];
                const size_t m = count[k + 1] - count[k];
                uint32_t maxa = 0;
                for (size_t q = 0; q < m; ++q) maxa = std::max(maxa, first[q].a & ~kItemSegment);
                if (maxa < (1u << 16)) {
                    std::vector<size_t> pos((size_t)maxa + 2, 0);
                    for (size_t q = 0; q < m; ++q) ++pos[(size_t)(maxa - (first[q].a & ~kItemSegment)) + 1];
                    for (size_t v = 0; v <= maxa; ++v) pos[v + 1] += pos[v];
                    std::vector<Item> tmp(first, first + m);
                    for (size_t q = 0; q < m; ++q) first[pos[(size_t)(maxa - (tmp[q].a & ~kItemSegment))]++] = tmp[q];
                } else {
                    std::stable_sort(first, first + m, [](const Item &a, const Item &b) { return a.a > b.a; });
                }
            }
            const size_t wg_first = wg;
            if (kid == kKidSeg) {
                for (size_t q = count[k]; q < count[k + 1]; q += kSegPerWg) {
                    const size_t m = std::min<size_t>(kSegPerWg, count[k + 1] - q);
                    for (size_t t = 0; t < m; ++t) out.items[q + t].b = t == 0 ? (uint32_t)m : 0u;
                    out.wg_item[wg++] = (uint32_t)q;
                }
            } else {
                for (size_t q = count[k]; q < count[k + 1]; ++q) {
                    const uint32_t wgs = out.items[q].b;
                    out.items[q].b = (uint32_t)(wg - wg_level);
                    std::fill(out.wg_item.begin() + wg, out.wg_item.begin() + wg + wgs, (uint32_t)q);
                    wg += wgs;
                }
            }
            out.launches.push_back({level, kid, count[k], count[k + 1] - count[k], wg_first, wg - wg_first, wg_level, bytes[k]});
        }
    out.wg_item.resize(wg);
}

void level_groups(const Schedule &sc, const LevelRouteOpts &o, std::vector<LaunchGroup> &out) {
    group_launches(sc, o.split_kinds, [&](int kid) { return route_of(kid, o); }, out);
}

}
```

sorobn_amd/csrc/planner.h:

```cpp
#pragma once
#include <array>
#include <cstdint>
#include <functional>
#include <memory>
#include <string>
#include <vector>

#include "emit_core.h"
#include "wave_plan.h"

namespace mibn {

struct Network {
    int n_vars = 0;
    std::vector<int32_t> card;
    std::vector<double> log2card;
    std::vector<std::vector<int32_t>> scope;
    std::vector<std::vector<int64_t>> cstride;
    std::vector<int64_t> pool_off;
    std::vector<int64_t> cells;
    std::vector<double> pool;
    std::vector<Bits> anc;
    std::vector<int32_t> depth;
    std::vector<std::vector<int32_t>> hints;
    std::vector<std::vector<int32_t>> hint_sorted;
    std::vector<int32_t> topo_asc, topo_desc;
    std::vector<B2> anc2, scope2, fam2;
    B2 multi2;
    int32_t uniform_log2 = -1;
    std::vector<int32_t> hint_flat;
    OrderNet order_view() const;
    std::vector<int32_t> scope_off32, scope_flat;
    std::vector<int64_t> cstride_flat;
    std::vector<uint64_t> anc_flat;
    EmitNet emit_view() const;
    bool wave_view(WNet &w) const;
    int nw = 1;
    int small_cells = 1024;
    int64_t big_iters = 4096;
    int tile_h = 0;
    int64_t tile_bytes = 512 << 10;
    double minfill_above = 2e7;
    int prune = 1;
    int outer = 1;
    int fuse = 1;
    int plan_cache = 1;
    uint64_t version = 0;
    mutable std::shared_ptr<void> templates;
    int chain = 1;
    int stagger = 1;
    int sweep = 5;
    int sweep_min = 2;
    int sweep_iters = kSweepItersDefault;
    int sweep_adapt = 4096;
    int builtin_sweeps = 1;
    int order_effort = 0;
    double second_above = 1e7;
    int order_weights = 1;
    int sweep_canon = 1;

    std::string set(int32_t n, const int32_t *card_, const int64_t *scope_off, const int32_t *scope_vars,
                    const int64_t *value_off, const double *values);
    void set_hints(int32_t n_hints, const int32_t *priorities);
};

enum class ProgramKind : uint8_t { Sum, Raw, Max, Draw, Map };
constexpr bool takes_query(ProgramKind k) { return k == ProgramKind::Sum || k == ProgramKind::Raw || k == ProgramKind::Map; }
constexpr bool never_prunes(ProgramKind k) { return k == ProgramKind::Max; }
constexpr bool step_wise(ProgramKind k) { return k == ProgramKind::Max || k == ProgramKind::Draw || k == ProgramKind::Map; }
constexpr bool may_use_templates(ProgramKind k) { return k == ProgramKind::Sum; }
constexpr bool allows_no_query(ProgramKind k) { return k == ProgramKind::Raw || k == ProgramKind::Map; }

struct Request {
    int32_t nq = 0, ne = 0;
    const int32_t *qvars = nullptr;
    const int32_t *evars = nullptr;
    const int32_t *ecodes = nullptr;
    int64_t out_off = 0;
    ProgramKind kind = ProgramKind::Sum;
    bool no_prune = false;
    const uint8_t *order = nullptr;
    int32_t n_order = -1;
    int32_t nl = 0;
    const int32_t *lvars = nullptr;
};

struct PlanStats {
    double alg_bytes = 0, alg_flops = 0, n_steps = 0, max_step_cells = 0;
    int64_t arena_cells = 0;
    int64_t out_cells = 0;
    int64_t argmax_cells = 0;
    int64_t kept_cells = 0;
    std::vector<int32_t> *order = nullptr;
};


MIBN_HD inline uint64_t record_offset(const uint32_t *p) {
    const uint32_t n_steps = p[0];
    uint64_t off = 1;
    for (uint32_t s = 0; s < n_steps; ++s) off += p[off + 6];
    return off;
}

struct ProgBuf {
    uint32_t *data = nullptr;
    size_t size = 0, cap = 0;
    uint32_t *(*grow)(void *ctx, uint32_t *old, size_t used, size_t new_cap) = nullptr;
    void *ctx = nullptr;
    uint32_t *extend(size_t words);
    void push(uint32_t w) { *extend(1) = w; }
    void release();
};

std::string plan_request(const Network &net, const Request &rq, ProgBuf &prog, PlanStats &st);
std::string emit_error_message(int err);
std::string plan_request(const Network &net, const Request &rq, std::vector<uint32_t> &prog, PlanStats &st);

class ThreadPool {
public:
    explicit ThreadPool(int n);
    ~ThreadPool();
    int size() const { return n_; }
    void run(const std::function<void(int)> &job);
private:
    struct Impl;
    Impl *impl_;
    int n_;
};

struct BatchPlan {
    std::vector<std::vector<Tag>> tags;
    std::vector<uint32_t> tag_first, tag_count;
    std::vector<size_t> thread_words;
    std::vector<uint64_t> prog_off;
    std::vector<double> cost;
    std::vector<int64_t> arena_need;
    std::vector<int32_t> thread_of;
    std::vector<uint64_t> local_off;
    int64_t arena_cells = 0;
    size_t total_words = 0;
    PlanStats st;
    std::string err;
};
void plan_batch(const Network &net, ThreadPool &pool, std::vector<ProgBuf> &bufs, int64_t b0, int64_t b1,
                const int64_t *q_off, const int32_t *q_vars, const int64_t *e_off, const int32_t *e_vars,
                const int32_t *e_codes, const int64_t *out_off, const char *skip, BatchPlan &bp, bool no_prune = false,
                const uint8_t *orders = nullptr, const int32_t *order_len = nullptr,
                int64_t out_first = -1,
                ProgramKind kind = ProgramKind::Sum,
                const int64_t *l_off = nullptr, const int32_t *l_vars = nullptr);

void estimate_costs(const Network &net, ThreadPool &pool, int64_t B, const int64_t *q_off, const int32_t *q_vars,
                    const int64_t *e_off, const int32_t *e_vars, double *cost);

struct Item {
    uint32_t req;
    uint32_t rel_off;
    uint32_t a, b;
};
constexpr int kSegPerWg = 4;
struct Launch {
    int level, kid;
    size_t first, count;
    size_t wg_first;
    size_t grid;
    size_t wg_level;
    double alg_bytes;
};
const char *kernel_name(int kid);

struct Schedule {
    std::vector<Item> items;
    std::vector<uint32_t> wg_item;
    std::vector<Launch> launches;
    std::vector<uint64_t> arena_off;
    int64_t arena_cells = 0;
    int n_levels = 0;
};
void build_schedule(const Network &net, const BatchPlan &bp, const std::vector<ProgBuf> &bufs, int64_t r0, int64_t r1,
                    Schedule &out);

struct LevelRouteOpts { bool split_kinds, seg_kernel, mfma_kernel, sweep_dma; };
enum class LevelRoute { Level, SweepDma, SweepReg, Segment, Mfma };
constexpr int kNumLevelRoutes = 5;
constexpr int kKidMfma1Cx4 = kKidFiber0 + 4, kKidMfma1Cx16 = kKidFiber0 + 6 + 4;
constexpr bool is_mfma1_class(int kid) { return kid == kKidMfma1Cx4 || kid == kKidMfma1Cx16; }
constexpr LevelRoute route_of(int kid, const LevelRouteOpts &o) {
    if (kid == kKidSweep) return o.sweep_dma ? LevelRoute::SweepDma : LevelRoute::SweepReg;
    if (o.split_kinds) return LevelRoute::Level;
    if (o.seg_kernel && kid == kKidSeg) return LevelRoute::Segment;
    if (o.mfma_kernel && is_mfma1_class(kid)) return LevelRoute::Mfma;
    return LevelRoute::Level;
}
struct LaunchGroup {
    LevelRoute route; int level, stat_kid;
    size_t wg_level, wg_first, grid; double alg_bytes; size_t first_launch, n_launches;
};
template <class RouteOf>
void group_launches(const Schedule &sc, bool each_alone, RouteOf &&route, std::vector<LaunchGroup> &out) {
    out.clear();
    for (size_t li = 0; li < sc.launches.size(); ++li) {
        const Launch &L = sc.launches[li];
        const LevelRoute r = route(L.kid);
        if (each_alone || out.empty() || out.back().level != L.level || out.back().route != r)
            out.push_back({r, L.level, each_alone ? L.kid : -1, L.wg_level, L.wg_first, 0, 0.0, li, 0});
        LaunchGroup &g = out.back();
        g.grid += L.grid; g.alg_bytes += L.alg_bytes; ++g.n_launches;
    }
}
void level_groups(const Schedule &sc, const LevelRouteOpts &o, std::vector<LaunchGroup> &out);

std::string validate_request(const Network &net, const Request &rq);
bool request_is_valid(const Network &net, const Request &rq);
std::string validate_mpe_request(const Network &net, const Request &rq);

}
```

sorobn_amd/csrc/sweep_kernel.hip.h:

```cpp
#pragma once
#include <hip/hip_runtime.h>

#include "planner.h"
#include "ve_kernel.hip.h"

namespace mibn {

constexpr int kSweepLdsBytes = kSweepTileCells * 8 + kSweepMaxT * 8 + kMaxStepWords * 4;

__device__ __forceinline__ int sweep_perm(const int c, const int kout, const int rb, const uint32_t surv) {
    int idx = c >> (2 * kout);
#pragma unroll
    for (int q = 0; q < 5; ++q)
        if (q < kout) idx += ((c >> (2 * q)) & 3) << (rb + 2 * (int)((surv >> (4 * q)) & 15));
    return idx;
}

template <int COUT, int SX, int SL>
__device__ __forceinline__ void sweep_fibers(double *__restrict__ L, const double *__restrict__ T, const int base, const int sx_,
                                             const int sl_, const int toff, const int loop_ts) {
    const int sx = SX ? SX : sx_, sl = SL ? SL : sl_;
    double t[4 * COUT];
#pragma unroll
    for (int l = 0; l < 4; ++l) {
        if (l == 0 || loop_ts) {
            const double *__restrict__ Tp = T + (toff + l * loop_ts);
#pragma unroll
            for (int q = 0; q < 4 * COUT; ++q) t[q] = Tp[q];
        }
        const int b = base + l * sl;
        double f[4];
#pragma unroll
        for (int x = 0; x < 4; ++x) f[x] = L[b + x * sx];
#pragma unroll
        for (int n = 0; n < COUT; ++n) {
            double s = f[0] * t[n];
#pragma unroll
            for (int x = 1; x < 4; ++x) s = __builtin_fma(f[x], t[n + COUT * x], s);
            L[b + n * sx] = s;
        }
    }
}

struct SweepTables {
    double *T;
    const uint32_t *stw, *smw;
    const double *pool;
    const double *slot;
    int k, t_total;
};
template <int WG>
__device__ __forceinline__ void sweep_build_tables_n(const SweepTables &b, const int tid) {
    for (int t = tid; t < b.t_total; t += WG) {
        int j = 0, rec0 = 0;
        while (j + 1 < b.k && t >= (int)((b.stw[j * kSweepStageWords + 1] & 0xffff) + (b.stw[j * kSweepStageWords + 1] >> 16))) {
            rec0 += (int)((b.stw[j * kSweepStageWords] >> 8) & 15);
            ++j;
        }
        const uint32_t s0 = b.stw[j * kSweepStageWords], s1 = b.stw[j * kSweepStageWords + 1];
        const int cout = (s0 >> 4) & 15, ns = (s0 >> 8) & 15;
        const int e = t - (int)(s1 & 0xffff);
        const int n = cout == 4 ? (e & 3) : 0;
        const int r = cout == 4 ? (e >> 2) : e;
        const int x = r & 3, c0 = (r >> 2) & 3, c1 = (r >> 4) & 3, c2 = (r >> 6) & 3;
        double v = 1.0;
        for (int i = 0; i < ns; ++i) {
            const uint32_t *rec = b.smw + (rec0 + i) * kSweepSmallWords;
            const int off = n * (int)rec[2] + x * (int)rec[3] + c0 * (int)rec[4] + c1 * (int)rec[5] + c2 * (int)rec[6];
            v *= table_ptr(rec[0], rec[1], b.pool, b.slot)[off];
        }
        b.T[t] = v;
    }
}
__device__ __forceinline__ void sweep_build_tables(const SweepTables &b, const int tid) { sweep_build_tables_n<kSweepWG>(b, tid); }

__device__ __forceinline__ void sweep_stage_lane(const uint32_t s0, const uint32_t s1, const uint32_t (&cw)[3], const int rb, const int tid,
                                                 int &base, int &toff) {
    const int nctrl = (s0 >> 12) & 15, loop = (s0 >> 16) & 15;
    base = tid & ((1 << rb) - 1);
    int bits = tid >> rb;
#pragma unroll
    for (int f = 0; f < 3; ++f) {
        const int fd = (s0 >> (20 + 4 * f)) & 15;
        if (fd != 7) {
            base += (bits & 3) << (rb + 2 * fd);
            bits >>= 2;
        }
    }
    toff = (int)(s1 & 0xffff);
#pragma unroll
    for (int c = 0; c < 3; ++c)
        if (c < nctrl) {
            const int src = cw[c] & 0xff, ts = (int)(cw[c] >> 8);
            if (src < 8 && src != loop) toff += ((base >> (rb + 2 * src)) & 3) * ts;
        }
}

template <int K>
__device__ __forceinline__ void sweep_tiles_impl(double *__restrict__ L, const double *__restrict__ T, const uint32_t *stw, const int k_rt,
                                                 const int rb_rt, const double *__restrict__ F, double *__restrict__ outp,
                                                 const long Rcells, const int t_begin, const int t_end, const int kout,
                                                 const uint32_t surv, const int tid, const SweepTables &tb) {
    constexpr int KS = K ? K : 5;
    const int k = K ? K : k_rt, rb = K ? 13 - 2 * K : rb_rt;
    const int Rt = 1 << rb;
    uint32_t sw0[KS], sw1[KS], swc[KS][3];
    int base[KS], toff0[KS];
#pragma unroll
    for (int j = 0; j < KS; ++j) {
        sw0[j] = sw1[j] = swc[j][0] = swc[j][1] = swc[j][2] = 0;
        base[j] = toff0[j] = 0;
        if (j < k) {
            sw0[j] = (uint32_t)uni((int)stw[j * kSweepStageWords]);
            sw1[j] = (uint32_t)uni((int)stw[j * kSweepStageWords + 1]);
#pragma unroll
            for (int c = 0; c < 3; ++c) swc[j][c] = (uint32_t)uni((int)stw[j * kSweepStageWords + 2 + c]);
            sweep_stage_lane(sw0[j], sw1[j], swc[j], rb, tid, base[j], toff0[j]);
        }
    }
    const int ocells = Rt << (2 * kout);
    const int p_tid2 = sweep_perm(2 * tid, kout, rb, surv);
    const int st0 = kout > 0 ? 1 << (rb + 2 * (int)(surv & 15)) : 1;
    const int rp = tid & ((Rt >> 1) - 1);
    const long g_tid = (long)(tid >> (rb - 1)) * Rcells + 2 * rp;
    const long g_step = (long)(kSweepWG >> (rb - 1)) * Rcells;
    double v[16];
    {
        const double *__restrict__ Ft = F + (long)t_begin * Rt + g_tid;
#pragma unroll
        for (int i = 0; i < 8; ++i) {
            const double2 q = *reinterpret_cast<const double2 *>(Ft + i * g_step);
            v[2 * i] = q.x;
            v[2 * i + 1] = q.y;
        }
    }
    sweep_build_tables(tb, tid);
    for (int tile = t_begin; tile < t_end; ++tile) {
        __syncthreads();
#pragma unroll
        for (int i = 0; i < 8; ++i) *reinterpret_cast<double2 *>(L + 2 * (i * kSweepWG + tid)) = make_double2(v[2 * i], v[2 * i + 1]);
        __syncthreads();
        const int rg = tile * Rt + (tid & (Rt - 1));
#define MIBN_SWEEP_STAGE(J)                                                                                                   \
        if (J < KS && J < k) {                                                                                                \
            constexpr int JJ = J < KS ? J : 0;                                                                                \
            const uint32_t s0 = sw0[JJ];                                                                                      \
            const int cout = (s0 >> 4) & 15, nctrl = (s0 >> 12) & 15, loop = (s0 >> 16) & 15;                                 \
            int toff = toff0[JJ], loop_ts = 0;                                                                                \
            _Pragma("unroll") for (int c = 0; c < 3; ++c)                                                                     \
                if (c < nctrl) {                                                                                              \
                    const int src = swc[JJ][c] & 0xff, ts = (int)(swc[JJ][c] >> 8);                                           \
                    if (src >= 8) toff += ((rg >> (src - 8)) & 3) * ts;                                                       \
                    else if (src == loop) loop_ts = ts;                                                                       \
                }                                                                                                             \
            constexpr int kRt = K ? (1 << (13 - 2 * (K ? K : 5))) : 0;                                                         \
            constexpr int kDig = K > J ? K - 1 - J : 0;                                                                       \
            constexpr int SX = K > J ? (kRt << (2 * kDig)) : 0;                                                               \
            constexpr int SL = K > J ? (kRt << (2 * sweep_loop_digit(K ? K : 5, kDig))) : 0;                                  \
            const int sx = 1 << (rb + 2 * (int)(s0 & 15)), sl = 1 << (rb + 2 * loop);                                         \
            if (cout == 4) sweep_fibers<4, SX, SL>(L, T, base[JJ], sx, sl, toff, loop_ts);                                    \
            else sweep_fibers<1, SX, SL>(L, T, base[JJ], sx, sl, toff, loop_ts);                                              \
            __syncthreads();                                                                                                  \
        }
        MIBN_SWEEP_STAGE(0)
        MIBN_SWEEP_STAGE(1)
        MIBN_SWEEP_STAGE(2)
        MIBN_SWEEP_STAGE(3)
        MIBN_SWEEP_STAGE(4)
#undef MIBN_SWEEP_STAGE
        {
            const long more = tile + 1 < t_end ? 1 : 0;
            const double *__restrict__ Ft = F + (long)(tile + more) * Rt + more * g_tid;
            const long g_step_ = more * g_step;
#pragma unroll
            for (int i = 0; i < 8; ++i) {
                const double2 q = *reinterpret_cast<const double2 *>(Ft + i * g_step_);
                v[2 * i] = q.x;
                v[2 * i + 1] = q.y;
            }
        }
        double *__restrict__ ot = outp + (long)tile * ocells;
#pragma unroll
        for (int i = 0; i < 8; ++i) {
            const int c0 = i * 2 * kSweepWG;
            if (c0 < ocells) {
                const int c = c0 + 2 * tid;
                if (c < ocells) {
                    const int a = sweep_perm(c0, kout, rb, surv) + p_tid2;
                    *reinterpret_cast<double2 *>(ot + c) = make_double2(L[a], L[a + st0]);
                }
            }
        }
    }
}

template <int K>
__device__ __forceinline__ void sweep_tiles(double *__restrict__ L, const double *__restrict__ T, const uint32_t *stw, const double *__restrict__ F,
                                         double *__restrict__ outp, const long Rcells, const int t_begin, const int t_end, const int kout,
                                         const uint32_t surv, const int tid, const SweepTables &tb) {
    sweep_tiles_impl<K>(L, T, stw, K, 13 - 2 * K, F, outp, Rcells, t_begin, t_end, kout, surv, tid, tb);
}

__device__ __forceinline__ void sweep_tiles_any(double *__restrict__ L, const double *__restrict__ T, const uint32_t *stw, const int k, const int rb,
                                                const double *__restrict__ F, double *__restrict__ outp, const long Rcells, const int t_begin,
                                                const int t_end, const int kout, const uint32_t surv, const int tid, const SweepTables &tb) {
    sweep_build_tables(tb, tid);
    const int Rt = 1 << rb;
    const int ocells = Rt << (2 * kout);
    const int rp = tid & ((Rt >> 1) - 1);
    const long g_tid = (long)(tid >> (rb - 1)) * Rcells + 2 * rp;
    const long g_step = (long)(kSweepWG >> (rb - 1)) * Rcells;
    for (int tile = t_begin; tile < t_end; ++tile) {
        __syncthreads();
        const double *__restrict__ Ft = F + (long)tile * Rt + g_tid;
#pragma unroll
        for (int i = 0; i < 8; ++i) *reinterpret_cast<double2 *>(L + 2 * (i * kSweepWG + tid)) = *reinterpret_cast<const double2 *>(Ft + i * g_step);
        __syncthreads();
        const int rg = tile * Rt + (tid & (Rt - 1));
        for (int j = 0; j < k; ++j) {
            const uint32_t s0 = (uint32_t)uni((int)stw[j * kSweepStageWords]), s1 = (uint32_t)uni((int)stw[j * kSweepStageWords + 1]);
            uint32_t cw[3];
#pragma unroll
            for (int c = 0; c < 3; ++c) cw[c] = (uint32_t)uni((int)stw[j * kSweepStageWords + 2 + c]);
            int base, toff;
            sweep_stage_lane(s0, s1, cw, rb, tid, base, toff);
            const int cout = (s0 >> 4) & 15, nctrl = (s0 >> 12) & 15, loop = (s0 >> 16) & 15;
            int loop_ts = 0;
#pragma unroll
            for (int c = 0; c < 3; ++c)
                if (c < nctrl) {
                    const int src = cw[c] & 0xff, ts = (int)(cw[c] >> 8);
                    if (src >= 8) toff += ((rg >> (src - 8)) & 3) * ts;
                    else if (src == loop) loop_ts = ts;
                }
            const int sx = 1 << (rb + 2 * (int)(s0 & 15)), sl = 1 << (rb + 2 * loop);
            if (cout == 4) sweep_fibers<4, 0, 0>(L, T, base, sx, sl, toff, loop_ts);
            else sweep_fibers<1, 0, 0>(L, T, base, sx, sl, toff, loop_ts);
            __syncthreads();
        }
        double *__restrict__ ot = outp + (long)tile * ocells;
        for (int c = tid; c < ocells; c += kSweepWG) ot[c] = L[sweep_perm(c, kout, rb, surv)];
    }
}


#ifndef MIBN_SWEEP_TAIL_LOCAL
#define MIBN_SWEEP_TAIL_LOCAL 1
#endif
#ifndef MIBN_SWEEP_DEAD_TAIL
#define MIBN_SWEEP_DEAD_TAIL 1
#endif
#ifndef MIBN_SWEEP_DEAD_SKIP
#define MIBN_SWEEP_DEAD_SKIP 1
// ... 235 lines not shown
    for (int l = 0; l < 2; ++l)
#pragma unroll
        for (int x = 0; x < 4; ++x) f[l][x] = Lp[(l * SL + x * SX) / 2];
    __builtin_amdgcn_fence(__ATOMIC_RELEASE, "wavefront");
    __builtin_amdgcn_wave_barrier();
    __builtin_amdgcn_fence(__ATOMIC_ACQUIRE, "wavefront");
    asm volatile("s_waitcnt lgkmcnt(0)" ::: "memory");
    dma_next();
    const bool lane_on = dead == 1 ? d1 == 0 : (dead == 2 ? d2 == 0 : (dead == 3 ? d3 == 0 : (dead == 4 ? h == 0 : true)));
    const int c_hi = (d1 << q1) + (d2 << q2) + (d3 << q3) + ((2 * h) << q4) + ((2 * rp) << 8);
    if (dead != 0) {
        if (!lane_on) return;
        double t0[16];
#pragma unroll
        for (int l = 0; l < 2; ++l) {
            if (dead == 4 && l == 1) break;
            double s0[4], s1v[4];
            if (PAR || l == 0 || loop_ts) {
                const double2 *__restrict__ Tp = reinterpret_cast<const double2 *>(T + (toff + l * loop_ts));
#pragma unroll
                for (int q = 0; q < 8; ++q) { const double2 v = Tp[q]; t0[2 * q] = v.x; t0[2 * q + 1] = v.y; }
            }
#pragma unroll
            for (int n = 0; n < 4; ++n) {
                s0[n] = f[l][0].x * t0[n];
#pragma unroll
                for (int x = 1; x < 4; ++x) s0[n] = __builtin_fma(f[l][x].x, t0[n + 4 * x], s0[n]);
            }
            if constexpr (PAR) {
                const double2 *__restrict__ Tq = reinterpret_cast<const double2 *>(T + (toff + l * loop_ts + par_ts));
#pragma unroll
                for (int q = 0; q < 8; ++q) { const double2 v = Tq[q]; t0[2 * q] = v.x; t0[2 * q + 1] = v.y; }
            }
#pragma unroll
            for (int n = 0; n < 4; ++n) {
                s1v[n] = f[l][0].y * t0[n];
#pragma unroll
                for (int x = 1; x < 4; ++x) s1v[n] = __builtin_fma(f[l][x].y, t0[n + 4 * x], s1v[n]);
            }
            {
                double *__restrict__ o0 = ot + (c_hi + (l << q4));
                double *__restrict__ o1 = o0 + (1 << 8);
                *reinterpret_cast<double2 *>(o0) = make_double2(s0[0], s0[1]);
                *reinterpret_cast<double2 *>(o0 + 2) = make_double2(s0[2], s0[3]);
                *reinterpret_cast<double2 *>(o1) = make_double2(s1v[0], s1v[1]);
                *reinterpret_cast<double2 *>(o1 + 2) = make_double2(s1v[2], s1v[3]);
            }
        }
    } else {
        double t0[4];
#pragma unroll
        for (int l = 0; l < 2; ++l) {
            if (PAR || l == 0 || loop_ts) {
                const double2 *__restrict__ Tp = reinterpret_cast<const double2 *>(T + (toff + l * loop_ts));
#pragma unroll
                for (int q = 0; q < 2; ++q) { const double2 v = Tp[q]; t0[2 * q] = v.x; t0[2 * q + 1] = v.y; }
            }
            double s0 = f[l][0].x * t0[0];
#pragma unroll
            for (int x = 1; x < 4; ++x) s0 = __builtin_fma(f[l][x].x, t0[x], s0);
            if constexpr (PAR) {
                const double2 *__restrict__ Tq = reinterpret_cast<const double2 *>(T + (toff + l * loop_ts + par_ts));
#pragma unroll
                for (int q = 0; q < 2; ++q) { const double2 v = Tq[q]; t0[2 * q] = v.x; t0[2 * q + 1] = v.y; }
            }
            double s1v = f[l][0].y * t0[0];
#pragma unroll
            for (int x = 1; x < 4; ++x) s1v = __builtin_fma(f[l][x].y, t0[x], s1v);
            double *__restrict__ o0 = ot + (c_hi + (l << q4));
            o0[0] = s0;
            o0[1 << 8] = s1v;
        }
    }
}

__device__ __forceinline__ int sweep_readout_cell(const int e, const int kout) {
    if (kout < 2) return 2 * e;
    const int mr = 2 * kout - 1;
    const int lo = e & 3, r3 = (e >> 2) & 7, hi = e >> 5;
    const int mid = hi & ((1 << (mr - 2)) - 1), top = hi >> (mr - 2);
    return 2 * (lo | (mid << 2) | (r3 << mr) | (top << (mr + 3)));
}

template <int K, bool OWN, bool DEAD = false, bool LOADER = false>
__device__ __forceinline__ void sweep_tiles_dma(double *__restrict__ L, double *__restrict__ T, const uint32_t *stw, const int k_rt,
                                                const int rb_rt, const double *__restrict__ F, double *__restrict__ outp,
                                                const long Rcells, const int t_begin, const int t_end, const int kout,
                                                const uint32_t surv, const int tid, const SweepTables &tb, const int dead = -1) {
    static_assert(!DEAD || (OWN && K == 5), "one dead digit: the wave-owned tail of a five-variable pass");
    constexpr int WG = kSweepWG;
    constexpr int KS = K ? K : 5;
    constexpr int PER = kSweepTileCells / 2 / WG;
    const int k = K ? K : k_rt, rb = K ? 13 - 2 * K : rb_rt;
    const int Rt = 1 << rb;
    const int ocells = Rt << (2 * kout);
    const int c_lane = sweep_readout_cell(tid, kout);
    const int p_lane = sweep_perm(c_lane, kout, rb, surv);
    const int st0 = kout > 0 ? 1 << (rb + 2 * (int)(surv & 15)) : 1;
    const int c_wave = uni(sweep_readout_cell(tid & ~63, kout));
    const int lane = tid & 63, wv = tid >> 6;
    const int own_rho0 = K == 5 ? (wv & 3) + 8 * (wv >> 2) : 2 * (wv >> 2) + 4 * (wv & 3);
    constexpr int kOwnRhoStep = K == 5 ? 4 : 1;
    const int rp = tid & ((Rt >> 1) - 1);
    const long g_tid = OWN ? (long)((512 * own_rho0 + 2 * lane) >> rb) * Rcells + ((2 * lane) & (Rt - 1))
                           : (long)(tid >> (rb - 1)) * Rcells + 2 * rp;
    const long g_step = (long)(WG >> (rb - 1)) * Rcells;
    const uint32_t lds_l = lds_byte_addr(L);
    auto dma_tile = [&](const int tile) {
        long g_lane = g_tid;
        if constexpr (!OWN) {
            int t2 = tid;
            asm volatile("" : "+v"(t2));
            g_lane = (long)(t2 >> (rb - 1)) * Rcells + 2 * (t2 & ((Rt >> 1) - 1));
        }
        const double *__restrict__ Ft = F + (long)tile * Rt + g_lane;
        if constexpr (OWN) {
            const uint32_t lb = (uint32_t)uni((int)(lds_l + 8u * 512u * (uint32_t)own_rho0));
#pragma unroll
            for (int i = 0; i < PER; ++i) {
                const int lam = 512 * kOwnRhoStep * (i >> 2) + 128 * (i & 3);
                dma16(Ft + (long)(lam >> rb) * Rcells, lb + (uint32_t)(8 * lam));
            }
        } else {
            const uint32_t lb = (uint32_t)uni((int)(lds_l + 16u * (uint32_t)(tid & ~63)));
#pragma unroll
            for (int i = 0; i < PER; ++i) dma16(Ft + i * g_step, lb + (uint32_t)(i * WG * 16));
        }
    };
    const int n_tiles = t_end - t_begin;
    double *__restrict__ const Lbase = L;
    if constexpr (LOADER) {
        static_assert(!LOADER || (K == 5 && OWN && !DEAD), "the loader experiment covers the canonical five-variable pass");
        if (tid >= WG) {
            auto fill = [&](const int tile, const int slot) {
                const uint32_t lb = (uint32_t)uni((int)(lds_l + 8u * (uint32_t)(slot * kSweepTileCells)));
                const double *__restrict__ Ft = F + (long)tile * Rt + ((2 * lane) & (Rt - 1));
#pragma unroll 8
                for (int j = 0; j < kSweepTileCells / 128; ++j) dma16(Ft + (long)((128 * j + 2 * lane) >> rb) * Rcells, lb + (uint32_t)(8 * 128 * j));
            };
            fill(t_begin, 0);
            for (int i = 0; i < n_tiles; ++i) {
                asm volatile("s_waitcnt vmcnt(0)" ::: "memory");
                __syncthreads();
                if (i + 1 < n_tiles) fill(t_begin + i + 1, (i + 1) & 1);
                __syncthreads();
            }
            return;
        }
    }
    MIBN_PROF_INIT
    if constexpr (!LOADER) dma_tile(t_begin);
    sweep_build_tables(tb, tid);
    for (int i = 0; i < n_tiles; ++i) {
        const int tile = t_begin + i;
        if constexpr (LOADER) L = Lbase + (i & 1) * kSweepTileCells;
        MIBN_PROF_TICK(0)
        static_assert(MIBN_SWEEP_VMCNT == 0 || MIBN_SWEEP_VMCNT == kSweepOwnTailStores, "the wait must leave exactly the tail's stores in flight");
        if constexpr (LOADER) {}
        else if (OWN && !DEAD && MIBN_SWEEP_VMCNT == kSweepOwnTailStores && i > 0) asm volatile("s_waitcnt vmcnt(%0)" ::"n"(kSweepOwnTailStores) : "memory");
        else asm volatile("s_waitcnt vmcnt(0)" ::: "memory");
        MIBN_PROF_TICK(1)
        __syncthreads();
        const int rg = tile * Rt + (K ? 2 * rp : (tid & (Rt - 1)));
#define MIBN_SWEEP_STAGE(J)                                                                                                   \
        if (J < KS && J < k && !(OWN && J == K - 1)) {                                                                        \
            const uint32_t s0 = (uint32_t)uni((int)stw[J * kSweepStageWords]), s1 = (uint32_t)uni((int)stw[J * kSweepStageWords + 1]); \
            uint32_t cw[3];                                                                                                   \
            _Pragma("unroll") for (int c = 0; c < 3; ++c) cw[c] = (uint32_t)uni((int)stw[J * kSweepStageWords + 2 + c]);      \
            constexpr SweepGeom G = sweep_geom(K > J ? K : 5, K > J ? J : 0);                                                 \
            const int cout = (s0 >> 4) & 15, nctrl = (s0 >> 12) & 15, loop = K > J ? G.loop : (int)((s0 >> 16) & 15);         \
            int bs, toff, loop_ts = 0, par_ts = 0;                                                                            \
            if constexpr (K > J) {     \
                bs = sweep_pair_base<(K > J ? K : 5), (K > J ? J : 0)>(tid);                                                  \
                toff = (int)(s1 & 0xffff);                                                                                    \
                _Pragma("unroll") for (int c = 0; c < 3; ++c)                                                                 \
                    if (c < nctrl) {                                                                                          \
                        const int src = cw[c] & 0xff, ts = (int)(cw[c] >> 8);                                                 \
                        if (src < 8) toff += ((bs >> (rb + 2 * src)) & 3) * ts;                    \
                    }                                                                                                         \
            } else {                                                                                                          \
                sweep_stage_lane(s0, s1, cw, rb, tid, bs, toff);                                                              \
            }                                                                                                                 \
            _Pragma("unroll") for (int c = 0; c < 3; ++c)                                                                     \
                if (c < nctrl) {                                                                                              \
                    const int src = cw[c] & 0xff, ts = (int)(cw[c] >> 8);                                                     \
                    if (src >= 8) { toff += ((rg >> (src - 8)) & 3) * ts; if (src == 8) par_ts = ts; }                        \
                    else if (src == loop) loop_ts = ts;                                                                       \
                }                                                                                                             \
            if constexpr (K > J) {                                                                                            \
                constexpr int kRt = 1 << (13 - 2 * (K ? K : 5));                                                               \
                constexpr int SX = kRt << (2 * G.dig), SL = kRt << (2 * G.loop);                                              \
                          \
                bool alive = true;                                                                                            \
                int nl = 2;                                                                                                   \
                if constexpr (DEAD) {                                                                                         \
                    if (MIBN_SWEEP_DEAD_SKIP && G.dig < dead) {                                                               \
                        if (dead == G.loop) { alive = ((bs >> (rb + 2 * G.loop + 1)) & 1) == 0; nl = 1; }                     \
                        else alive = ((bs >> (rb + 2 * dead)) & 3) == 0;                                                      \
                    }                                                                                                         \
                }                                                                                                             \
                if (alive) {                                                                                                  \
                    if (cout == 4) sweep_fiber_pairs<4, SX, SL>(L, T, bs, toff, loop_ts, par_ts, nl);                         \
                    else sweep_fiber_pairs<1, SX, SL>(L, T, bs, toff, loop_ts, par_ts, nl);                                   \
                }                                                                                                             \
                        \
                if constexpr (G.sync_after && !(MIBN_SWEEP_TAIL_LOCAL && OWN && J == K - 2)) __syncthreads();                 \
                else {          \
                    __builtin_amdgcn_fence(__ATOMIC_RELEASE, "wavefront");                                                    \
                    __builtin_amdgcn_wave_barrier();                                                                          \
                    __builtin_amdgcn_fence(__ATOMIC_ACQUIRE, "wavefront");                                                    \
                }                                                                                                             \
            } else {                                                                                                          \
                const int sx = 1 << (rb + 2 * (int)(s0 & 15)), sl = 1 << (rb + 2 * loop);                                     \
                if (cout == 4) sweep_fibers<4, 0, 0>(L, T, bs, sx, sl, toff, loop_ts);                                        \
                else sweep_fibers<1, 0, 0>(L, T, bs, sx, sl, toff, loop_ts);                                                  \
                __syncthreads();                                                                                              \
            }                                                                                                                 \
            MIBN_PROF_TICK(2 + J)                                                                                             \
        }
        MIBN_SWEEP_STAGE(0)
        MIBN_SWEEP_STAGE(1)
        MIBN_SWEEP_STAGE(2)
        MIBN_SWEEP_STAGE(3)
        MIBN_SWEEP_STAGE(4)
#undef MIBN_SWEEP_STAGE
        double *__restrict__ ot = outp + (long)tile * ocells;
        if constexpr (OWN) {
            constexpr int JL = K > 0 ? K - 1 : 0;
            const uint32_t s1 = (uint32_t)uni((int)stw[JL * kSweepStageWords + 1]);
            const int nctrl = (int)(((uint32_t)uni((int)stw[JL * kSweepStageWords]) >> 12) & 15);
            uint32_t cw[3];
#pragma unroll
            for (int c = 0; c < 3; ++c) cw[c] = (uint32_t)uni((int)stw[JL * kSweepStageWords + 2 + c]);
            bool par = false;
#pragma unroll
            for (int c = 0; c < 3; ++c) par = par || (c < nctrl && (cw[c] & 0xff) == 8);
            auto dma_next = [&]() { if constexpr (!LOADER) { if (i + 1 < n_tiles) dma_tile(tile + 1); } };
            if constexpr (DEAD) {
                if (par) sweep_last_stage_out_dead<true>(L, T, ot, tid, tile * Rt, s1, cw, nctrl, dead, dma_next);
                else sweep_last_stage_out_dead<false>(L, T, ot, tid, tile * Rt, s1, cw, nctrl, dead, dma_next);
            } else {
                if (par) sweep_last_stage_out<(K > 0 ? K : 5), true>(L, T, ot, tid, tile * Rt, s1, cw, nctrl, dma_next);
                else sweep_last_stage_out<(K > 0 ? K : 5), false>(L, T, ot, tid, tile * Rt, s1, cw, nctrl, dma_next);
            }
            MIBN_PROF_TICK(7)
        } else {
#pragma unroll
            for (int q = 0; q < PER; ++q) {
                const int c_trip = sweep_readout_cell(q * WG, kout);
                if (c_trip + c_wave < ocells) {
                    const int c = c_trip + c_lane;
                    const int a = sweep_perm(c_trip, kout, rb, surv) + p_lane;
                    if (c < ocells) *reinterpret_cast<double2 *>(ot + c) = make_double2(L[a], L[a + st0]);
                }
            }
            MIBN_PROF_TICK(7)
            if (i + 1 < n_tiles) {
                __syncthreads();
                dma_tile(tile + 1);
            }
        }
        MIBN_PROF_TICK(8)
    }
    MIBN_PROF_END
}

__global__ __launch_bounds__(kSweepWG, 4) void ve_sweep_dma_kernel(const LevelArgs A) {
    extern __shared__ __attribute__((aligned(16))) double sweep_lds[];
    double *__restrict__ L = sweep_lds;
    double *__restrict__ T = sweep_lds + kSweepTileCells;
    uint32_t *sh_step = reinterpret_cast<uint32_t *>(sweep_lds + kSweepTileCells + kSweepMaxT);
    const int tid = threadIdx.x;
    const uint32_t wg = blockIdx.x + A.wg_base;
    const Item it = A.items[A.wg_item[wg]];
    double *__restrict__ slot = A.arena + A.arena_off[it.req];
    const uint32_t *p = A.prog + A.prog_off[it.req] + it.rel_off;
    const int words = (int)p[6];
    for (int i = tid; i < words; i += kSweepWG) sh_step[i] = p[i];
    __syncthreads();
    const int k = uni((int)((sh_step[0] >> 16) & 0xff)), rb = uni((int)((sh_step[0] >> 24) & 0xff));
    const int tiles = uni((int)sh_step[3]);
    const int kout = uni((int)(sh_step[7] & 0xffff)), t_total = uni((int)(sh_step[7] >> 16));
    const uint32_t surv = (uint32_t)uni((int)sh_step[8]);
    const long Rcells = (long)tiles << rb;
    const uint32_t *stw = sh_step + kHdrWords + 2;
    const uint32_t *smw = stw + k * kSweepStageWords;
    const double *__restrict__ F = slot + ((uint64_t)sh_step[kHdrWords] | ((uint64_t)sh_step[kHdrWords + 1] << 32));
    double *__restrict__ outp = slot + ((uint64_t)sh_step[4] | ((uint64_t)sh_step[5] << 32));
    const SweepTables tb{T, stw, smw, A.pool, slot, k, t_total};
    const int t_begin = (int)((wg - it.b) * it.a);
    const int t_end = min(tiles, t_begin + (int)it.a);
    const bool canon = (sh_step[1] >> 16) & kFlagSweepCanon;
    int dead = -1;
    if (MIBN_SWEEP_DEAD_TAIL && canon && k == 5 && kout == 4) {
        const uint32_t packs[5] = {0x4321u, 0x4320u, 0x4310u, 0x4210u, 0x3210u};
#pragma unroll
        for (int d = 0; d < 5; ++d)
            if (surv == packs[d]) dead = d;
    }
    if (canon && k == 5 && kout == 5 && surv == 0x43210u) sweep_tiles_dma<5, true>(L, T, stw, 5, 3, F, outp, Rcells, t_begin, t_end, kout, surv, tid, tb);
    else if (dead >= 0) sweep_tiles_dma<5, true, true>(L, T, stw, 5, 3, F, outp, Rcells, t_begin, t_end, kout, surv, tid, tb, dead);
    else if (canon && k == 5) sweep_tiles_dma<5, false>(L, T, stw, 5, 3, F, outp, Rcells, t_begin, t_end, kout, surv, tid, tb);
    else if (canon && k == 4 && kout == 4 && surv == 0x3210u) sweep_tiles_dma<4, true>(L, T, stw, 4, 5, F, outp, Rcells, t_begin, t_end, kout, surv, tid, tb);
    else if (canon && k == 4) sweep_tiles_dma<4, false>(L, T, stw, 4, 5, F, outp, Rcells, t_begin, t_end, kout, surv, tid, tb);
    else if (canon && k == 3) sweep_tiles_dma<3, false>(L, T, stw, 3, 7, F, outp, Rcells, t_begin, t_end, kout, surv, tid, tb);
    else if (canon && k == 2) sweep_tiles_dma<2, false>(L, T, stw, 2, 9, F, outp, Rcells, t_begin, t_end, kout, surv, tid, tb);
    else sweep_tiles_dma<0, false>(L, T, stw, k, rb, F, outp, Rcells, t_begin, t_end, kout, surv, tid, tb);
}

constexpr int kSweepLoaderWG = kSweepWG + 64;
constexpr int kSweepLoaderLdsBytes = 2 * kSweepTileCells * 8 + kSweepMaxT * 8 + kMaxStepWords * 4;
__global__ __launch_bounds__(kSweepLoaderWG) void ve_sweep_loader_kernel(const LevelArgs A) {
    extern __shared__ __attribute__((aligned(16))) double sweep_lds[];
    double *__restrict__ L = sweep_lds;
    double *__restrict__ T = sweep_lds + 2 * kSweepTileCells;
    uint32_t *sh_step = reinterpret_cast<uint32_t *>(sweep_lds + 2 * kSweepTileCells + kSweepMaxT);
    const int tid = threadIdx.x;
    const uint32_t wg = blockIdx.x + A.wg_base;
    const Item it = A.items[A.wg_item[wg]];
    double *__restrict__ slot = A.arena + A.arena_off[it.req];
    const uint32_t *p = A.prog + A.prog_off[it.req] + it.rel_off;
    const int words = (int)p[6];
    for (int i = tid; i < words; i += kSweepLoaderWG) sh_step[i] = p[i];
    __syncthreads();
    const int k = uni((int)((sh_step[0] >> 16) & 0xff)), rb = uni((int)((sh_step[0] >> 24) & 0xff));
    const int tiles = uni((int)sh_step[3]);
    const int kout = uni((int)(sh_step[7] & 0xffff)), t_total = uni((int)(sh_step[7] >> 16));
    const uint32_t surv = (uint32_t)uni((int)sh_step[8]);
    const long Rcells = (long)tiles << rb;
    const uint32_t *stw = sh_step + kHdrWords + 2;
    const uint32_t *smw = stw + k * kSweepStageWords;
    const double *__restrict__ F = slot + ((uint64_t)sh_step[kHdrWords] | ((uint64_t)sh_step[kHdrWords + 1] << 32));
    double *__restrict__ outp = slot + ((uint64_t)sh_step[4] | ((uint64_t)sh_step[5] << 32));
    const SweepTables tb{T, stw, smw, A.pool, slot, k, t_total};
    const int t_begin = (int)((wg - it.b) * it.a);
    const int t_end = min(tiles, t_begin + (int)it.a);
    const bool canon = (sh_step[1] >> 16) & kFlagSweepCanon;
    if (canon && k == 5 && kout == 5 && surv == 0x43210u) sweep_tiles_dma<5, true, false, true>(L, T, stw, 5, 3, F, outp, Rcells, t_begin, t_end, kout, surv, tid, tb);
    (void)rb;
}

__global__ __launch_bounds__(kSweepWG, 4) void ve_sweep_kernel(const LevelArgs A) {
    extern __shared__ __attribute__((aligned(16))) double sweep_lds[];
    double *__restrict__ L = sweep_lds;
    double *__restrict__ T = sweep_lds + kSweepTileCells;
    uint32_t *sh_step = reinterpret_cast<uint32_t *>(sweep_lds + kSweepTileCells + kSweepMaxT);
    const int tid = threadIdx.x;
    const uint32_t wg = blockIdx.x + A.wg_base;
    const Item it = A.items[A.wg_item[wg]];
    double *__restrict__ slot = A.arena + A.arena_off[it.req];
    const uint32_t *p = A.prog + A.prog_off[it.req] + it.rel_off;
    const int words = (int)p[6];
    for (int i = tid; i < words; i += kSweepWG) sh_step[i] = p[i];
    __syncthreads();
    const int k = uni((int)((sh_step[0] >> 16) & 0xff)), rb = uni((int)((sh_step[0] >> 24) & 0xff));
    const int tiles = uni((int)sh_step[3]);
    const int kout = uni((int)(sh_step[7] & 0xffff)), t_total = uni((int)(sh_step[7] >> 16));
    const uint32_t surv = (uint32_t)uni((int)sh_step[8]);
    const long Rcells = (long)tiles << rb;
    const uint32_t *stw = sh_step + kHdrWords + 2;
    const uint32_t *smw = stw + k * kSweepStageWords;
    const double *__restrict__ F = slot + ((uint64_t)sh_step[kHdrWords] | ((uint64_t)sh_step[kHdrWords + 1] << 32));
    double *__restrict__ outp = slot + ((uint64_t)sh_step[4] | ((uint64_t)sh_step[5] << 32));
    const SweepTables tb{T, stw, smw, A.pool, slot, k, t_total};
    const int t_begin = (int)((wg - it.b) * it.a);
    const int t_end = min(tiles, t_begin + (int)it.a);
    const bool canon = (sh_step[1] >> 16) & kFlagSweepCanon;
    if (canon && k == 5) sweep_tiles<5>(L, T, stw, F, outp, Rcells, t_begin, t_end, kout, surv, tid, tb);
    else if (canon && k == 4) sweep_tiles<4>(L, T, stw, F, outp, Rcells, t_begin, t_end, kout, surv, tid, tb);
    else if (canon && k == 3) sweep_tiles<3>(L, T, stw, F, outp, Rcells, t_begin, t_end, kout, surv, tid, tb);
    else sweep_tiles_any(L, T, stw, k, rb, F, outp, Rcells, t_begin, t_end, kout, surv, tid, tb);
}

}
```

Baseline: 320,700.

## Fuse fiber-grow step into following sweep pass, computing tiles in LDS

Adds a grow-fuse path. An eligible fiber step whose output feeds a canonical five-variable sweep is no longer written to the arena. The sweep kernel instead rebuilds each input tile in LDS from the fiber's small tables and parent factor. Eligibility marks are computed on the device after emit, and on the host for fallback programs, and the scheduler packs the fused step's words into the item. This removes a global write and read of the large intermediate and one launch level, at the cost of extra per-tile arithmetic, LDS table space and more complex scheduling.

```diff
diff --git a/__graft_entry__.py b/__graft_entry__.py
--- a/__graft_entry__.py
+++ b/__graft_entry__.py
@@ -6,7 +6,7 @@
 CSRC = os.path.join(ROOT, "sorobn_amd", "csrc")
 LIB = os.path.join(ROOT, "sorobn_amd", "libmibn.so")
 SOURCES = [os.path.join(CSRC, f) for f in ("planner.cpp", "engine.hip")]
-DEPS = SOURCES + [os.path.join(CSRC, f) for f in ("planner.h", "plan_policy.h", "device_mem.h", "emit_core.h", "order_search.h", "ve_kernel.hip.h", "sweep_kernel.hip.h", "tiny_kernel.hip.h", "gibbs_kernel.hip.h", "sampler_plan.h",
+DEPS = SOURCES + [os.path.join(CSRC, f) for f in ("planner.h", "plan_policy.h", "device_mem.h", "emit_core.h", "grow_fuse.h", "order_search.h", "ve_kernel.hip.h", "sweep_kernel.hip.h", "tiny_kernel.hip.h", "gibbs_kernel.hip.h", "sampler_plan.h",
                                               "sample_kernel.hip.h", "count_kernel.hip.h", "wave_prims.h", "wave_plan.h", "wave_plan_kernel.hip.h", "elim_kernel.hip.h", "draw_kernel.hip.h", "expect_kernel.hip.h", "score_kernel.hip.h", "citest_kernel.hip.h", "likelihood_kernel.hip.h", "bp_plan.h", "bp_kernel.hip.h", "count_weighted_kernel.hip.h")] + \
     [os.path.join(ROOT, "include", "mibn.h")]
 
diff --git a/sorobn_amd/csrc/engine.hip b/sorobn_amd/csrc/engine.hip
--- a/sorobn_amd/csrc/engine.hip
+++ b/sorobn_amd/csrc/engine.hip
@@ -38,6 +38,31 @@
 #include "wave_plan_kernel.hip.h"
 
 using namespace mibn;
+
+struct GrowMarkArgs {
+    const uint32_t *prog;
+    uint32_t prog_stride, tag_cap;
+    const EmitMeta *meta;
+    const Tag *tags;
+    uint8_t *marks;
+    int64_t B;
+    int small_cells, min_tiles;
+};
+__global__ __launch_bounds__(256) void grow_mark_kernel(const GrowMarkArgs A) {
+    const int64_t i = (int64_t)blockIdx.x * 256 + threadIdx.x;
+    if (i >= A.B) return;
+    const EmitMeta m = A.meta[i];
+    if (m.err || m.n_tags < 2 || (uint64_t)m.tag_first + m.n_tags > A.tag_cap) return;
+    const uint32_t *p = A.prog + (size_t)i * A.prog_stride + m.prog_first;
+    Tag s = A.tags[m.tag_first];
+    for (uint32_t k = 0; k + 1 < m.n_tags; ++k) {
+        const Tag g = s;
+        s = A.tags[m.tag_first + k + 1];
+        if (grow_fuse_candidate(g, s) && (uint64_t)m.prog_first + s.rel_off + kMaxStepWords <= A.prog_stride &&
+            grow_fuse_eligible(p + g.rel_off, p + s.rel_off, A.small_cells, A.min_tiles, nullptr))
+            A.marks[m.tag_first + k] = 1;
+    }
+}
 
 namespace {
 double now_ms() {
@@ -379,6 +404,7 @@
     int threads = 0;
     int trace = 0;
     int split_kinds = 0;
+    int grow_fuse = 1;
     int overlap = 1;
     int sweep_dma = 1;
     int gibbs_lds = 1;
@@ -487,6 +513,7 @@
     auto *h = new mibn_ctx();
     h->net.order_effort = 1; h->net.second_above = h->pol.base_second_above;
     h->net.small_cells = kEngineSmallCells;
+    h->net.grow_fuse = h->grow_fuse;
     h->net.minfill_above = h->pol.base_minfill;
     h->planner_only = true;
     *out = h;
@@ -502,6 +529,7 @@
     auto *h = new mibn_ctx();
     h->net.order_effort = 1; h->net.second_above = h->pol.base_second_above;
     h->net.small_cells = kEngineSmallCells;
+    h->net.grow_fuse = h->grow_fuse;
     h->net.minfill_above = h->pol.base_minfill;
     h->device = device;
     if (hipSetDevice(device) != hipSuccess) { delete h; return MIBN_E_NODEVICE; }
@@ -547,6 +575,7 @@
     else if (n == "chunk_sets") { if (mibn_drain(h) != MIBN_OK) return MIBN_E_HIP; h->n_sets = std::max(2, std::min(kChunkSets, (int)value)); h->set_cursor = 0; }
     else if (n == "trace") h->trace = (int)value;
     else if (n == "split_kinds") h->split_kinds = value != 0;
+    else if (n == "grow_fuse") { h->grow_fuse = value != 0; h->net.grow_fuse = h->grow_fuse; }
     else if (n == "overlap") { if (mibn_drain(h) != MIBN_OK) return MIBN_E_HIP; h->overlap = value != 0; }
     else if (n == "sweep_dma") h->sweep_dma = value != 0;
     else if (n == "seg_kernel") h->seg_kernel = value != 0;
@@ -971,7 +1000,7 @@
         }
     }
     if ((rc = pinned(h, h->emit_in, in_bytes))) return rc;
-    if ((rc = pinned(h, h->emit_out, (size_t)n * sizeof(EmitMeta) + tag_cap * sizeof(Tag) + 64))) return rc;
+    if ((rc = pinned(h, h->emit_out, (size_t)n * sizeof(EmitMeta) + tag_cap * sizeof(Tag) + 64 + tag_cap))) return rc;
     if (!h->d_emit_cursor) HIP_TRY(h, h->d_emit_cursor.reset(16));
     if (!wave) {
     if ((rc = ensure(h, h->d_orders, (size_t)n * 128))) return rc;
@@ -1118,6 +1147,15 @@
         hipLaunchKernelGGL(emit_kernel, dim3((unsigned)((m + per_wg - 1) / per_wg)), dim3(64 * h->plan_waves), 0, P, A);
         HIP_TRY(h, hipGetLastError());
     }
+    if (h->net.grow_fuse) {
+        GrowMarkArgs G;
+        G.prog = st.d_prog; G.prog_stride = (uint32_t)stride; G.meta = meta_out; G.tags = tags_out;
+        G.marks = reinterpret_cast<uint8_t *>(tags_out + tag_cap);
+        G.B = n; G.tag_cap = (uint32_t)tag_cap; G.small_cells = h->net.small_cells; G.min_tiles = h->net.grow_fuse_min_tiles;
+        std::memset(G.marks, 0, tag_cap);
+        hipLaunchKernelGGL(grow_mark_kernel, dim3((unsigned)((n + 255) / 256)), dim3(256), 0, P, G);
+        HIP_TRY(h, hipGetLastError());
+    }
     HIP_TRY(h, hipEventRecord(h->emit_ev[1], P));
     return MIBN_OK;
 }
@@ -1146,11 +1184,14 @@
     ck.arena_need.assign(n, 0);
     ck.thread_of.assign(n, 0);
     ck.local_off.assign(n, 0);
+    ck.words_on_host.clear();
     ck.thread_words.clear();
     ck.tag_first.assign(n, 0);
     ck.tag_count.assign(n, 0);
     ck.tags.resize(1);
     ck.tags[0].assign(tags, tags + n_tags);
+    ck.tag_marks.assign(1, {});
+    if (h->net.grow_fuse) { const uint8_t *marks = reinterpret_cast<const uint8_t *>(tags + tag_cap); ck.tag_marks[0].assign(marks, marks + n_tags); }
     bool refused = false, beyond = false;
     for (int64_t i = 0; i < n; ++i) {
         const EmitMeta &m = meta[i];
@@ -1602,6 +1643,8 @@
     ck.tags.resize((size_t)T + 1);
     for (int t = 0; t < T; ++t) ck.tags[(size_t)t].swap(hp.tags[(size_t)t]);
     ck.tags[(size_t)T].swap(dp.tags[0]);
+    ck.tag_marks.assign((size_t)T + 1, {});
+    if (!dp.tag_marks.empty()) ck.tag_marks[(size_t)T].swap(dp.tag_marks[0]);
     ck.thread_words = hp.thread_words;
     auto join = [&](auto &dst, const auto &a, const auto &b) { dst.assign(a.begin(), a.end()); dst.insert(dst.end(), b.begin(), b.end()); };
     join(ck.cost, dp.cost, hp.cost);
@@ -1609,6 +1652,8 @@
     join(ck.tag_first, dp.tag_first, hp.tag_first);
     join(ck.tag_count, dp.tag_count, hp.tag_count);
     join(ck.local_off, dp.local_off, hp.local_off);
+    ck.words_on_host.assign((size_t)nd, 0);
+    ck.words_on_host.insert(ck.words_on_host.end(), hp.words_on_host.begin(), hp.words_on_host.end());
     ck.thread_of.assign((size_t)nd, T);
     ck.thread_of.insert(ck.thread_of.end(), hp.thread_of.begin(), hp.thread_of.end());
     const size_t prog_base = (size_t)nd * stride;
@@ -1631,6 +1676,8 @@
     const size_t X = ck.tags.size();
     ck.tags.resize(X + xp.tags.size());
     for (size_t t = 0; t < xp.tags.size(); ++t) ck.tags[X + t] = xp.tags[t];
+    ck.tag_marks.resize(ck.tags.size());
+    for (size_t t = 0; t < xp.tags.size(); ++t) ck.tag_marks[X + t].assign(h->net.grow_fuse ? xp.tags[t].size() : 0, 0);
     bool fits = true;
     for (int64_t i : beyond) {
         const uint32_t *w = st.xbufs[(size_t)xp.thread_of[(size_t)i]].data + xp.local_off[(size_t)i];
@@ -1643,6 +1690,9 @@
         ck.thread_of[(size_t)i] = (int32_t)(X + (size_t)xp.thread_of[(size_t)i]);
         ck.tag_first[(size_t)i] = xp.tag_first[(size_t)i];
         ck.tag_count[(size_t)i] = xp.tag_count[(size_t)i];
+        if (h->net.grow_fuse)
+            grow_fuse_mark(h->net, xp.tags[(size_t)xp.thread_of[(size_t)i]].data() + xp.tag_first[(size_t)i], xp.tag_count[(size_t)i], w,
+                           ck.tag_marks[X + (size_t)xp.thread_of[(size_t)i]].data() + xp.tag_first[(size_t)i]);
         ck.cost[(size_t)i] = xp.cost[(size_t)i];
         ck.arena_need[(size_t)i] = xp.arena_need[(size_t)i];
     }
@@ -1842,7 +1892,8 @@
     int rc;
     double t0 = now_ms();
     Schedule &sc = st.sched;
-    build_schedule(h->net, st.plan, st.bufs, r0, r1, sc);
+    build_schedule(h->net, st.plan, st.bufs, r0, r1, sc, !h->split_kinds);
+    h->stats.alg_bytes -= sc.grow_fuse_bytes;
     h->stats.plan_ms += now_ms() - t0;
     R.call_fixed_ms += now_ms() - t0;
     if (h->trace) std::fprintf(stderr, "[mibn plan] build_schedule %.2f ms (%zu items, %zu workgroups, %zu launches)\n", now_ms() - t0, sc.items.size(), sc.wg_item.size(), sc.launches.size());
diff --git a/sorobn_amd/csrc/grow_fuse.h b/sorobn_amd/csrc/grow_fuse.h
--- /dev/null
+++ b/sorobn_amd/csrc/grow_fuse.h
@@ -0,0 +1,145 @@
+#pragma once
+#include <cstdint>
+
+#include "emit_core.h"
+
+namespace mibn {
+
+constexpr uint32_t kItemGrowFuse = 1u << 30;
+constexpr int kItemGrowWordsShift = 8;
+constexpr uint32_t kItemTilesMask = 0xff;
+static_assert(kTileMax <= (int)kItemTilesMask && kMaxStepWords < (1 << 16), "the fields of a fused item's Item::a");
+
+struct GrowDesc {
+    int na, ns, nN, nT, T;
+    const uint32_t *smalls;
+    const uint32_t *tcard;
+    const uint32_t *rax;
+    const int32_t *bst;
+    uint64_t f_off;
+    int xs;
+};
+
+MIBN_HD inline GrowDesc grow_desc(const uint32_t *g) {
+    GrowDesc d;
+    d.na = (int)((g[0] >> 16) & 0xff);
+    d.ns = (int)((g[7] >> 4) & 0xf);
+    d.nN = (int)((g[7] >> 8) & 0xf);
+    d.nT = d.nN + (int)((g[7] >> 12) & 0xf);
+    d.T = (int)(g[8] & 0xffff);
+    const uint32_t *q = g + kHdrWords;
+    d.f_off = (uint64_t)q[0] | ((uint64_t)q[1] << 32);
+    d.xs = (int)q[2];
+    q += 4;
+    d.smalls = q;
+    q += d.ns * (4 + d.nT);
+    d.tcard = q;
+    q += d.nT + 16;
+    d.rax = q;
+    q += 3 * d.na;
+    d.bst = (const int32_t *)q;
+    return d;
+}
+
+template <class Table>
+MIBN_HD inline double grow_table_entry(const GrowDesc &d, const int t, Table table) {
+    const int rn = t & 15, x = (t >> 4) & 3, r = t >> 6;
+    double v = 1.0;
+    for (int j = 0; j < d.ns; ++j) {
+        const uint32_t *rec = d.smalls + j * (4 + d.nT);
+        const int32_t *sts = (const int32_t *)(rec + 4);
+        int off = x * (int)rec[2];
+        int a = rn, c = r;
+        for (int k = 0; k < d.nN; ++k) { const int cd = (int)d.tcard[k]; const int qq = a / cd; off += (a - qq * cd) * sts[k]; a = qq; }
+        for (int k = d.nN; k < d.nT; ++k) { const int cd = (int)d.tcard[k]; const int qq = c / cd; off += (c - qq * cd) * sts[k]; c = qq; }
+        v *= table(rec[0], rec[1])[off];
+    }
+    return v;
+}
+
+MIBN_HD inline void grow_offsets(const GrowDesc &d, const uint32_t rho, int &foff, int &toff) {
+    foff = 0;
+    toff = 0;
+    for (int a = 0; a < d.na; ++a) {
+        const uint32_t card = d.rax[3 * a];
+        if (card > 1) {
+            const int dg = (int)((rho >> (__builtin_ctz(d.rax[3 * a + 1]) - 4)) & (card - 1));
+            foff += dg * d.bst[a];
+            toff += dg * (int)d.rax[3 * a + 2];
+        }
+    }
+}
+
+MIBN_HD inline uint32_t grow_rho_of_tile(const int tile) { return (uint32_t)(tile >> 1); }
+MIBN_HD inline uint32_t grow_rho_of_xc(const int xc, const int tiles) { return (uint32_t)xc * (uint32_t)(tiles >> 1); }
+
+MIBN_HD inline void grow_fill8(const double (&f)[4], const double *Tq, double (&out)[8]) {
+    for (int j = 0; j < 8; ++j) {
+        double s = f[0] * Tq[j];
+        for (int x = 1; x < 4; ++x) s = __builtin_fma(f[x], Tq[j + 16 * x], s);
+        out[j] = s;
+    }
+}
+
+constexpr int kGrowRejectKinds = 1, kGrowRejectClass = 2, kGrowRejectSweep = 3, kGrowRejectTiles = 4, kGrowRejectNotInput = 5, kGrowRejectLayout = 6,
+              kGrowRejectLds = 7, kGrowRejectOverlap = 8, kGrowRejectReasons = 9;
+MIBN_HD inline int grow_fuse_reject(const uint32_t *g, const uint32_t *s, const int small_cells, const int min_tiles, int64_t *g_cells) {
+    if ((g[0] & 0xff) != kKindFiber || (s[0] & 0xff) != kKindSweep) return kGrowRejectKinds;
+    const uint64_t g_out = (uint64_t)g[4] | ((uint64_t)g[5] << 32);
+    const uint64_t s_in = (uint64_t)s[kHdrWords] | ((uint64_t)s[kHdrWords + 1] << 32);
+    if (s_in != g_out || (s_in & kConstFlag)) return kGrowRejectNotInput;
+    const uint32_t gf = g[1] >> 16, sf = s[1] >> 16;
+    if ((gf & (kFlagFinal | kFlagOuter | kFlagChain)) || !(gf & kFlagContig) || !((g[1] >> kRowStrideShift) & 0xff)) return kGrowRejectClass;
+    if ((g[7] & 0xf) != 1 || (g[7] >> 16) != 16 || (g[1] & 0xffff) != 4 || (g[8] >> 16) != 4) return kGrowRejectClass;
+    if (!(sf & kFlagSweepCanon) || ((s[0] >> 16) & 0xff) != 5 || ((s[0] >> 24) & 0xff) != 3) return kGrowRejectSweep;
+    const int64_t tiles = (int64_t)s[3];
+    if (tiles < 2 || tiles < min_tiles || (tiles & (tiles - 1))) return kGrowRejectTiles;
+    const int64_t G = tiles * kSweepTileCells;
+    if ((int64_t)g[2] * (int64_t)g[3] * 16 != G || G > (int64_t(1) << 31)) return kGrowRejectLayout;
+    const GrowDesc d = grow_desc(g);
+    if (d.f_off & kConstFlag) return kGrowRejectLayout;
+    if (d.xs < 0 || d.nN < 1) return kGrowRejectLayout;
+    for (int n = 0; n < 16; ++n)
+        if (d.tcard + d.nT + n >= g + g[6] || d.tcard[d.nT + n] != (uint32_t)n) return kGrowRejectLayout;
+    if ((const uint32_t *)(d.bst + d.na) > g + g[6]) return kGrowRejectLayout;
+    uint64_t mask = 0;
+    int64_t f_span = 3 * (int64_t)d.xs + 1;
+    for (int a = 0; a < d.na; ++a) {
+        const uint64_t card = d.rax[3 * a], ost = d.rax[3 * a + 1];
+        if (card == 0 || (card & (card - 1))) return kGrowRejectLayout;
+        if (card == 1) continue;
+        if (ost < 16 || (ost & (ost - 1)) || d.bst[a] < 0 || (int32_t)d.rax[3 * a + 2] < 0) return kGrowRejectLayout;
+        const uint64_t field = (card - 1) * ost;
+        if (mask & field) return kGrowRejectLayout;
+        mask |= field;
+        f_span += (int64_t)(card - 1) * d.bst[a];
+    }
+    if (mask != (uint64_t)(G - 16)) return kGrowRejectLayout;
+    if (f_span > (int64_t(1) << 31)) return kGrowRejectLayout;
+    const int t_total = (int)(s[7] >> 16);
+    if (((t_total + 1) & ~1) + d.T > kSweepMaxT || (d.T & 63)) return kGrowRejectLds;
+    if (g[6] + s[6] > (uint32_t)kMaxStepWords) return kGrowRejectLds;
+    const int kout = (int)(s[7] & 0xffff);
+    const uint64_t so = (uint64_t)s[4] | ((uint64_t)s[5] << 32);
+    const uint64_t so_end = so + (uint64_t)tiles * ((uint64_t)8 << (2 * kout));
+    auto under_output = [&](const uint64_t b, const uint64_t e) { return b < so_end && so < e; };
+    if (under_output(d.f_off, d.f_off + (uint64_t)f_span)) return kGrowRejectOverlap;
+    for (int j = 0; j < d.ns; ++j) {
+        const uint32_t *rec = d.smalls + j * (4 + d.nT);
+        const uint64_t off = (uint64_t)rec[0] | ((uint64_t)rec[1] << 32);
+        if (off & kConstFlag) continue;
+        const int32_t *sts = (const int32_t *)(rec + 4);
+        int64_t span = 1 + 3 * (int64_t)(int32_t)rec[2];
+        bool plain = (int32_t)rec[2] >= 0;
+        for (int k = 0; k < d.nT; ++k) { plain = plain && sts[k] >= 0; span += (int64_t)(d.tcard[k] - 1) * sts[k]; }
+        if (!plain) span = small_cells;
+        if (under_output(plain ? off : off - (uint64_t)small_cells, off + (uint64_t)span)) return kGrowRejectOverlap;
+    }
+    if (g_cells) *g_cells = G;
+    return 0;
+}
+MIBN_HD inline bool grow_fuse_eligible(const uint32_t *g, const uint32_t *s, const int small_cells, const int min_tiles, int64_t *g_cells) {
+    return grow_fuse_reject(g, s, small_cells, min_tiles, g_cells) == 0;
+}
+
+}
diff --git a/sorobn_amd/csrc/planner.cpp b/sorobn_amd/csrc/planner.cpp
--- a/sorobn_amd/csrc/planner.cpp
+++ b/sorobn_amd/csrc/planner.cpp
@@ -1222,6 +1222,8 @@
     ck.arena_need.assign(n, 0);
     ck.thread_of.assign(n, 0);
     ck.local_off.assign(n, 0);
+    ck.words_on_host.assign(n, 1);
+    ck.tag_marks.clear();
     ck.thread_words.assign(T, 0);
     ck.tag_first.assign(n, 0);
     ck.tag_count.assign(n, 0);
@@ -1424,10 +1426,17 @@
 constexpr ClassOrder kClassOrder;
 static_assert(kClassOrder.routes_contiguous(), "the classes of a kernel must be contiguous in the class order: level_groups merges neighbours only");
 
+void grow_fuse_mark(const Network &net, const Tag *tg, uint32_t cnt, const uint32_t *prog, uint8_t *marks) {
+    for (uint32_t k = 0; k < cnt; ++k)
+        marks[k] = k + 1 < cnt && grow_fuse_candidate(tg[k], tg[k + 1]) &&
+                   grow_fuse_eligible(prog + tg[k].rel_off, prog + tg[k + 1].rel_off, net.small_cells, net.grow_fuse_min_tiles, nullptr);
+}
+
 void build_schedule(const Network &net, const BatchPlan &bp, const std::vector<ProgBuf> &bufs, int64_t r0, int64_t r1,
-                    Schedule &out) {
-    (void)bufs;
+                    Schedule &out, bool allow_grow_fuse) {
     const int64_t n = r1 - r0;
+    out.n_grow_fused = 0;
+    out.grow_fuse_bytes = 0;
     out.items.clear();
     out.wg_item.clear();
     out.launches.clear();
@@ -1440,12 +1449,67 @@
     out.arena_cells = top;
     int n_levels = 0;
     size_t n_tags = 0, n_wg = 0;
-    for (int64_t i = 0; i < n; ++i) {
-        const int64_t r = r0 + i;
-        const Tag *tg = bp.tags[bp.thread_of[r]].data() + bp.tag_first[r];
-        const uint32_t cnt = bp.tag_count[r];
-        if (cnt) n_levels = std::max(n_levels, (int)tg[cnt - 1].level + 1);
-        n_tags += cnt;
+    std::vector<uint8_t> fz;
+    std::vector<uint16_t> lv;
+    std::vector<uint32_t> gw;
+    std::vector<float> fb;
+    if (net.grow_fuse && allow_grow_fuse) {
+        size_t t0 = 0, total = 0;
+        for (int64_t i = 0; i < n; ++i) total += bp.tag_count[r0 + i];
+        for (int64_t i = 0; i < n; ++i) {
+            const int64_t r = r0 + i;
+            const uint32_t cnt = bp.tag_count[r];
+            const size_t w = (size_t)bp.thread_of[r];
+            const uint8_t *marks = w < bp.tag_marks.size() && !bp.tag_marks[w].empty() && bp.tag_marks[w].size() == bp.tags[w].size()
+                                       ? bp.tag_marks[w].data() + bp.tag_first[r] : nullptr;
+            const bool words = !marks && (size_t)r < bp.words_on_host.size() && bp.words_on_host[(size_t)r] && w < bufs.size() && bufs[w].data;
+            if ((marks || words) && cnt > 1) {
+                const Tag *tg = bp.tags[w].data() + bp.tag_first[r];
+                const uint32_t *prog = words ? bufs[w].data + bp.local_off[r] : nullptr;
+                for (uint32_t k = 0; k < cnt; ++k) {
+                    if (k + 1 < cnt && grow_fuse_candidate(tg[k], tg[k + 1]) &&
+                        (marks ? marks[k] != 0
+                               : grow_fuse_eligible(prog + tg[k].rel_off, prog + tg[k + 1].rel_off, net.small_cells, net.grow_fuse_min_tiles, nullptr))) {
+                        const int64_t g_cells = (int64_t)tg[k + 1].a * kSweepTileCells;
+                        if (fz.empty()) { fz.assign(total, 0); lv.assign(total, 0); gw.assign(total, 0); fb.assign(total, 0.f); }
+                        fz[t0 + k] = 1;
+                        fz[t0 + k + 1] = 2;
+                        gw[t0 + k + 1] = tg[k + 1].rel_off - tg[k].rel_off;
+                        fb[t0 + k + 1] = (float)((double)tg[k].bytes + (double)tg[k + 1].bytes - 16.0 * (double)g_cells);
+                        ++out.n_grow_fused;
+                        out.grow_fuse_bytes += 16.0 * (double)g_cells;
+                        ++k;
+                    }
+                }
+            }
+            t0 += cnt;
+        }
+        if (!fz.empty()) {
+            t0 = 0;
+            for (int64_t i = 0; i < n; ++i) {
+                const int64_t r = r0 + i;
+                const Tag *tg = bp.tags[bp.thread_of[r]].data() + bp.tag_first[r];
+                const uint32_t cnt = bp.tag_count[r];
+                uint16_t dropped = 0;
+                for (uint32_t k = 0; k < cnt; ++k) {
+                    lv[t0 + k] = (uint16_t)(tg[k].level - dropped);
+                    if (fz[t0 + k] == 1) ++dropped;
+                }
+                t0 += cnt;
+            }
+        }
+    }
+    const bool fused = !fz.empty();
+    {
+        size_t t0 = 0;
+        for (int64_t i = 0; i < n; ++i) {
+            const int64_t r = r0 + i;
+            const Tag *tg = bp.tags[bp.thread_of[r]].data() + bp.tag_first[r];
+            const uint32_t cnt = bp.tag_count[r];
+            if (cnt) n_levels = std::max(n_levels, (int)(fused ? lv[t0 + cnt - 1] : tg[cnt - 1].level) + 1);
+            n_tags += cnt;
+            t0 += cnt;
+        }
     }
     const int G = std::max(1, std::min(net.stagger, 8));
     const int delta = G > 1 ? (n_levels + G - 1) / G : 0;
@@ -1456,15 +1520,19 @@
     std::vector<size_t> count(nb + 1, 0);
     std::vector<double> bytes(nb, 0.0);
     std::vector<uint64_t> sweep_tiles((size_t)n_levels, 0);
+    size_t tix = 0;
+    auto level_of = [&](const Tag &t, size_t x) { return (int)(fused ? lv[x] : t.level); };
     for (int64_t i = 0; i < n; ++i) {
         const int64_t r = r0 + i;
         const Tag *tg = bp.tags[bp.thread_of[r]].data() + bp.tag_first[r];
         const int sh = shift(i);
-        for (uint32_t k = 0; k < bp.tag_count[r]; ++k) {
-            const size_t bkt = (size_t)(tg[k].level + sh) * kNumKernels + kClassOrder.rank_of[tg[k].kid];
+        for (uint32_t k = 0; k < bp.tag_count[r]; ++k, ++tix) {
+            if (fused && fz[tix] == 1) continue;
+            const int level = level_of(tg[k], tix) + sh;
+            const size_t bkt = (size_t)level * kNumKernels + kClassOrder.rank_of[tg[k].kid];
             ++count[bkt + 1];
-            bytes[bkt] += tg[k].bytes;
-            if (tg[k].kid == kKidSweep) sweep_tiles[(size_t)(tg[k].level + sh)] += tg[k].a;
+            bytes[bkt] += fused && fz[tix] == 2 ? fb[tix] : tg[k].bytes;
+            if (tg[k].kid == kKidSweep) sweep_tiles[(size_t)level] += tg[k].a;
             else n_wg += tg[k].wgs;
         }
     }
@@ -1472,24 +1540,29 @@
     if (net.sweep_adapt)
         for (int l = 0; l < n_levels; ++l)
             while (sweep_iters[(size_t)l] > 2 && sweep_tiles[(size_t)l] / sweep_iters[(size_t)l] < (uint64_t)net.sweep_adapt) sweep_iters[(size_t)l] /= 2;
+    tix = 0;
     for (int64_t i = 0; i < n; ++i) {
         const int64_t r = r0 + i;
         const Tag *tg = bp.tags[bp.thread_of[r]].data() + bp.tag_first[r];
         const int sh = shift(i);
-        for (uint32_t k = 0; k < bp.tag_count[r]; ++k)
-            if (tg[k].kid == kKidSweep) { const uint32_t it = sweep_iters[(size_t)(tg[k].level + sh)]; n_wg += (tg[k].a + it - 1) / it; }
+        for (uint32_t k = 0; k < bp.tag_count[r]; ++k, ++tix)
+            if (tg[k].kid == kKidSweep) { const uint32_t it = sweep_iters[(size_t)(level_of(tg[k], tix) + sh)]; n_wg += (tg[k].a + it - 1) / it; }
     }
     for (size_t k = 0; k < nb; ++k) count[k + 1] += count[k];
-    out.items.resize(n_tags);
+    out.items.resize(n_tags - out.n_grow_fused);
+    tix = 0;
     std::vector<size_t> cur(count.begin(), count.end() - 1);
     for (int64_t i = 0; i < n; ++i) {
         const int64_t r = r0 + i;
         const Tag *tg = bp.tags[bp.thread_of[r]].data() + bp.tag_first[r];
         const int sh = shift(i);
-        for (uint32_t k = 0; k < bp.tag_count[r]; ++k) {
+        for (uint32_t k = 0; k < bp.tag_count[r]; ++k, ++tix) {
+            if (fused && fz[tix] == 1) continue;
+            const int level = level_of(tg[k], tix) + sh;
             uint32_t a = tg[k].a, wgs = tg[k].wgs;
-            if (tg[k].kid == kKidSweep) { const uint32_t it = sweep_iters[(size_t)(tg[k].level + sh)]; wgs = (a + it - 1) / it; a = it; }
-            out.items[cur[(size_t)(tg[k].level + sh) * kNumKernels + kClassOrder.rank_of[tg[k].kid]]++] = Item{(uint32_t)i, tg[k].rel_off, a, wgs};
+            if (tg[k].kid == kKidSweep) { const uint32_t it = sweep_iters[(size_t)level]; wgs = (a + it - 1) / it; a = it; }
+            if (fused && fz[tix] == 2) a |= kItemGrowFuse | (gw[tix] << kItemGrowWordsShift);
+            out.items[cur[(size_t)level * kNumKernels + kClassOrder.rank_of[tg[k].kid]]++] = Item{(uint32_t)i, tg[k].rel_off, a, wgs};
         }
     }
     out.wg_item.resize(n_wg);
diff --git a/sorobn_amd/csrc/planner.h b/sorobn_amd/csrc/planner.h
--- a/sorobn_amd/csrc/planner.h
+++ b/sorobn_amd/csrc/planner.h
@@ -7,6 +7,7 @@
 #include <vector>
 
 #include "emit_core.h"
+#include "grow_fuse.h"
 #include "wave_plan.h"
 
 namespace mibn {
@@ -58,6 +59,8 @@
     double second_above = 1e7;
     int order_weights = 1;
     int sweep_canon = 1;
+    int grow_fuse = 0;
+    int grow_fuse_min_tiles = 2;
 
     std::string set(int32_t n, const int32_t *card_, const int64_t *scope_off, const int32_t *scope_vars,
                     const int64_t *value_off, const double *values);
@@ -137,6 +140,8 @@
     std::vector<int64_t> arena_need;
     std::vector<int32_t> thread_of;
     std::vector<uint64_t> local_off;
+    std::vector<uint8_t> words_on_host;
+    std::vector<std::vector<uint8_t>> tag_marks;
     int64_t arena_cells = 0;
     size_t total_words = 0;
     PlanStats st;
@@ -176,15 +181,19 @@
     std::vector<uint64_t> arena_off;
     int64_t arena_cells = 0;
     int n_levels = 0;
+    size_t n_grow_fused = 0;
+    double grow_fuse_bytes = 0;
 };
 void build_schedule(const Network &net, const BatchPlan &bp, const std::vector<ProgBuf> &bufs, int64_t r0, int64_t r1,
-                    Schedule &out);
+                    Schedule &out, bool allow_grow_fuse = true);
 
 struct LevelRouteOpts { bool split_kinds, seg_kernel, mfma_kernel, sweep_dma; };
 enum class LevelRoute { Level, SweepDma, SweepReg, Segment, Mfma };
 constexpr int kNumLevelRoutes = 5;
 constexpr int kKidMfma1Cx4 = kKidFiber0 + 4, kKidMfma1Cx16 = kKidFiber0 + 6 + 4;
 constexpr bool is_mfma1_class(int kid) { return kid == kKidMfma1Cx4 || kid == kKidMfma1Cx16; }
+MIBN_HD inline bool grow_fuse_candidate(const Tag &g, const Tag &s) { return g.kid == kKidMfma1Cx4 && s.kid == kKidSweep && s.rel_off > g.rel_off; }
+void grow_fuse_mark(const Network &net, const Tag *tg, uint32_t cnt, const uint32_t *prog, uint8_t *marks);
 constexpr LevelRoute route_of(int kid, const LevelRouteOpts &o) {
     if (kid == kKidSweep) return o.sweep_dma ? LevelRoute::SweepDma : LevelRoute::SweepReg;
     if (o.split_kinds) return LevelRoute::Level;
diff --git a/sorobn_amd/csrc/sweep_kernel.hip.h b/sorobn_amd/csrc/sweep_kernel.hip.h
--- a/sorobn_amd/csrc/sweep_kernel.hip.h
+++ b/sorobn_amd/csrc/sweep_kernel.hip.h
@@ -1,12 +1,70 @@
 #pragma once
 #include <hip/hip_runtime.h>
 
+#include "grow_fuse.h"
 #include "planner.h"
 #include "ve_kernel.hip.h"
 
 namespace mibn {
 
 constexpr int kSweepLdsBytes = kSweepTileCells * 8 + kSweepMaxT * 8 + kMaxStepWords * 4;
+
+struct GrowFill {
+    const uint32_t *gw;
+    const double *T0;
+    const double *F;
+    int xs, half_tiles;
+};
+__device__ __forceinline__ GrowFill grow_fill_of(const uint32_t *gw, const double *T0, const double *slot, const int tiles) {
+    const uint64_t f_off = (uint64_t)(uint32_t)uni((int)gw[kHdrWords]) | ((uint64_t)(uint32_t)uni((int)gw[kHdrWords + 1]) << 32);
+    return GrowFill{gw, T0, slot + f_off, uni((int)gw[kHdrWords + 2]), tiles >> 1};
+}
+__device__ __forceinline__ void grow_build_table(const uint32_t *gw, double *__restrict__ T0, const double *pool, const double *slot, const int tid) {
+    const GrowDesc d = grow_desc(gw);
+    for (int t = tid; t < d.T; t += kSweepWG)
+        T0[t] = grow_table_entry(d, t, [&](const uint32_t lo, const uint32_t hi) { return table_ptr(lo, hi, pool, slot); });
+}
+__device__ __forceinline__ int grow_xc(const int tid, const int q) {
+    const int wv = tid >> 6;
+    return 64 * ((wv & 3) + 8 * (wv >> 2) + 4 * q) + (tid & 63);
+}
+__device__ __forceinline__ void grow_load(const GrowFill &g, const int tile, int tid, double (&f)[2][4], int (&to)[2]) {
+    asm volatile("" : "+v"(tid));
+    const int na = uni((int)((g.gw[0] >> 16) & 0xff)), ns = uni((int)((g.gw[7] >> 4) & 0xf));
+    const int nT = uni((int)(((g.gw[7] >> 8) & 0xf) + ((g.gw[7] >> 12) & 0xf)));
+    const uint32_t *rax = g.gw + (kHdrWords + 4 + 16) + ns * (4 + nT) + nT;
+    const int *bst = reinterpret_cast<const int *>(rax + 3 * na);
+    int fo[2];
+#pragma unroll
+    for (int q = 0; q < 2; ++q) {
+        const uint32_t rho = grow_rho_of_tile(tile) + grow_rho_of_xc(grow_xc(tid, q), 2 * g.half_tiles);
+        fo[q] = 0;
+        to[q] = 8 * (tile & 1);
+        for (int a = 0; a < na; ++a) {
+            const uint32_t card = (uint32_t)uni((int)rax[3 * a]);
+            if (card > 1) {
+                const int dg = (int)((rho >> (uni((int)__builtin_ctz(rax[3 * a + 1])) - 4)) & (card - 1));
+                fo[q] += dg * uni(bst[a]);
+                to[q] += dg * uni((int)rax[3 * a + 2]);
+            }
+        }
+    }
+#pragma unroll
+    for (int q = 0; q < 2; ++q)
+#pragma unroll
+        for (int x = 0; x < 4; ++x) f[q][x] = g.F[fo[q] + x * g.xs];
+}
+__device__ __forceinline__ void grow_store(const GrowFill &g, int tid, const double (&f)[2][4], const int (&to)[2], double *__restrict__ L) {
+    asm volatile("" : "+v"(tid));
+#pragma unroll
+    for (int q = 0; q < 2; ++q) {
+        double out[8];
+        grow_fill8(f[q], static_cast<const double *>(__builtin_assume_aligned(g.T0 + to[q], 16)), out);
+        double2 *__restrict__ Lp = reinterpret_cast<double2 *>(L + 8 * grow_xc(tid, q));
+#pragma unroll
+        for (int j = 0; j < 4; ++j) Lp[j] = make_double2(out[2 * j], out[2 * j + 1]);
+    }
+}
 
 __device__ __forceinline__ int sweep_perm(const int c, const int kout, const int rb, const uint32_t surv) {
     int idx = c >> (2 * kout);
@@ -40,6 +98,13 @@
             L[b + n * sx] = s;
         }
     }
+}
+
+__device__ __forceinline__ void grow_fill_tile(const GrowFill &g, const int tile, const int tid, double *__restrict__ L) {
+    double f[2][4];
+    int to[2];
+    grow_load(g, tile, tid, f, to);
+    grow_store(g, tid, f, to, L);
 }
 
 struct SweepTables {
@@ -96,11 +161,12 @@
         }
 }
 
-template <int K>
+template <int K, bool FUSED = false>
 __device__ __forceinline__ void sweep_tiles_impl(double *__restrict__ L, const double *__restrict__ T, const uint32_t *stw, const int k_rt,
                                                  const int rb_rt, const double *__restrict__ F, double *__restrict__ outp,
                                                  const long Rcells, const int t_begin, const int t_end, const int kout,
-                                                 const uint32_t surv, const int tid, const SweepTables &tb) {
+                                                 const uint32_t surv, const int tid, const SweepTables &tb, const uint32_t *gw = nullptr) {
+    static_assert(!FUSED || K == 5, "the fused fill: five-variable passes");
     constexpr int KS = K ? K : 5;
     const int k = K ? K : k_rt, rb = K ? 13 - 2 * K : rb_rt;
     const int Rt = 1 << rb;
@@ -125,7 +191,12 @@
     const long g_tid = (long)(tid >> (rb - 1)) * Rcells + 2 * rp;
     const long g_step = (long)(kSweepWG >> (rb - 1)) * Rcells;
     double v[16];
-    {
+    GrowFill gfill{};
+    if constexpr (FUSED) {
+        double *T0 = tb.T + ((tb.t_total + 1) & ~1);
+        gfill = grow_fill_of(gw, T0, tb.slot, (int)(Rcells >> 3));
+        grow_build_table(gw, T0, tb.pool, tb.slot, tid);
+    } else {
         const double *__restrict__ Ft = F + (long)t_begin * Rt + g_tid;
 #pragma unroll
         for (int i = 0; i < 8; ++i) {
@@ -137,8 +208,12 @@
     sweep_build_tables(tb, tid);
     for (int tile = t_begin; tile < t_end; ++tile) {
         __syncthreads();
-#pragma unroll
-        for (int i = 0; i < 8; ++i) *reinterpret_cast<double2 *>(L + 2 * (i * kSweepWG + tid)) = make_double2(v[2 * i], v[2 * i + 1]);
+        if constexpr (FUSED) {
+            grow_fill_tile(gfill, tile, tid, L);
+        } else {
+#pragma unroll
+            for (int i = 0; i < 8; ++i) *reinterpret_cast<double2 *>(L + 2 * (i * kSweepWG + tid)) = make_double2(v[2 * i], v[2 * i + 1]);
+        }
         __syncthreads();
         const int rg = tile * Rt + (tid & (Rt - 1));
 #define MIBN_SWEEP_STAGE(J)                                                                                                   \
@@ -168,7 +243,7 @@
         MIBN_SWEEP_STAGE(3)
         MIBN_SWEEP_STAGE(4)
 #undef MIBN_SWEEP_STAGE
-        {
+        if constexpr (!FUSED) {
             const long more = tile + 1 < t_end ? 1 : 0;
             const double *__restrict__ Ft = F + (long)(tile + more) * Rt + more * g_tid;
             const long g_step_ = more * g_step;
@@ -570,12 +645,14 @@
     return 2 * (lo | (mid << 2) | (r3 << mr) | (top << (mr + 3)));
 }
 
-template <int K, bool OWN, bool DEAD = false, bool LOADER = false>
+template <int K, bool OWN, bool DEAD = false, bool LOADER = false, bool FUSED = false>
 __device__ __forceinline__ void sweep_tiles_dma(double *__restrict__ L, double *__restrict__ T, const uint32_t *stw, const int k_rt,
                                                 const int rb_rt, const double *__restrict__ F, double *__restrict__ outp,
                                                 const long Rcells, const int t_begin, const int t_end, const int kout,
-                                                const uint32_t surv, const int tid, const SweepTables &tb, const int dead = -1) {
+                                                const uint32_t surv, const int tid, const SweepTables &tb, const int dead = -1,
+                                                const uint32_t *gw = nullptr) {
     static_assert(!DEAD || (OWN && K == 5), "one dead digit: the wave-owned tail of a five-variable pass");
+    static_assert(!FUSED || (K == 5 && !LOADER), "the fused fill: five-variable passes");
     constexpr int WG = kSweepWG;
     constexpr int KS = K ? K : 5;
     constexpr int PER = kSweepTileCells / 2 / WG;
@@ -637,14 +714,25 @@
         }
     }
     MIBN_PROF_INIT
+    GrowFill gfill{};
+    if constexpr (FUSED) {
+        double *T0 = T + ((tb.t_total + 1) & ~1);
+        gfill = grow_fill_of(gw, T0, tb.slot, (int)(Rcells >> 3));
+        grow_build_table(gw, T0, tb.pool, tb.slot, tid);
+        sweep_build_tables(tb, tid);
+        __syncthreads();
+        grow_fill_tile(gfill, t_begin, tid, L);
+    } else {
     if constexpr (!LOADER) dma_tile(t_begin);
     sweep_build_tables(tb, tid);
+    }
     for (int i = 0; i < n_tiles; ++i) {
         const int tile = t_begin + i;
         if constexpr (LOADER) L = Lbase + (i & 1) * kSweepTileCells;
         MIBN_PROF_TICK(0)
         static_assert(MIBN_SWEEP_VMCNT == 0 || MIBN_SWEEP_VMCNT == kSweepOwnTailStores, "the wait must leave exactly the tail's stores in flight");
         if constexpr (LOADER) {}
+        else if constexpr (FUSED) {}
         else if (OWN && !DEAD && MIBN_SWEEP_VMCNT == kSweepOwnTailStores && i > 0) asm volatile("s_waitcnt vmcnt(%0)" ::"n"(kSweepOwnTailStores) : "memory");
         else asm volatile("s_waitcnt vmcnt(0)" ::: "memory");
         MIBN_PROF_TICK(1)
@@ -723,7 +811,7 @@
             bool par = false;
 #pragma unroll
             for (int c = 0; c < 3; ++c) par = par || (c < nctrl && (cw[c] & 0xff) == 8);
-            auto dma_next = [&]() { if constexpr (!LOADER) { if (i + 1 < n_tiles) dma_tile(tile + 1); } };
+            auto dma_next = [&]() { if constexpr (!LOADER && !FUSED) { if (i + 1 < n_tiles) dma_tile(tile + 1); } };
             if constexpr (DEAD) {
                 if (par) sweep_last_stage_out_dead<true>(L, T, ot, tid, tile * Rt, s1, cw, nctrl, dead, dma_next);
                 else sweep_last_stage_out_dead<false>(L, T, ot, tid, tile * Rt, s1, cw, nctrl, dead, dma_next);
@@ -731,6 +819,7 @@
                 if (par) sweep_last_stage_out<(K > 0 ? K : 5), true>(L, T, ot, tid, tile * Rt, s1, cw, nctrl, dma_next);
                 else sweep_last_stage_out<(K > 0 ? K : 5), false>(L, T, ot, tid, tile * Rt, s1, cw, nctrl, dma_next);
             }
+            if constexpr (FUSED) { if (i + 1 < n_tiles) grow_fill_tile(gfill, tile + 1, tid, L); }
             MIBN_PROF_TICK(7)
         } else {
 #pragma unroll
@@ -745,7 +834,8 @@
             MIBN_PROF_TICK(7)
             if (i + 1 < n_tiles) {
                 __syncthreads();
-                dma_tile(tile + 1);
+                if constexpr (FUSED) grow_fill_tile(gfill, tile + 1, tid, L);
+                else dma_tile(tile + 1);
             }
         }
         MIBN_PROF_TICK(8)
@@ -764,7 +854,9 @@
     double *__restrict__ slot = A.arena + A.arena_off[it.req];
     const uint32_t *p = A.prog + A.prog_off[it.req] + it.rel_off;
     const int words = (int)p[6];
-    for (int i = tid; i < words; i += kSweepWG) sh_step[i] = p[i];
+    const int gwords = uni((int)((it.a & kItemGrowFuse) ? (it.a >> kItemGrowWordsShift) & 0xffff : 0u));
+    const int it_tiles = (int)(it.a & kItemTilesMask);
+    for (int i = tid; i < words + gwords; i += kSweepWG) sh_step[i] = i < words ? p[i] : (p - gwords)[i - words];
     __syncthreads();
     const int k = uni((int)((sh_step[0] >> 16) & 0xff)), rb = uni((int)((sh_step[0] >> 24) & 0xff));
     const int tiles = uni((int)sh_step[3]);
@@ -776,8 +868,8 @@
     const double *__restrict__ F = slot + ((uint64_t)sh_step[kHdrWords] | ((uint64_t)sh_step[kHdrWords + 1] << 32));
     double *__restrict__ outp = slot + ((uint64_t)sh_step[4] | ((uint64_t)sh_step[5] << 32));
     const SweepTables tb{T, stw, smw, A.pool, slot, k, t_total};
-    const int t_begin = (int)((wg - it.b) * it.a);
-    const int t_end = min(tiles, t_begin + (int)it.a);
+    const int t_begin = (int)(wg - it.b) * it_tiles;
+    const int t_end = min(tiles, t_begin + it_tiles);
     const bool canon = (sh_step[1] >> 16) & kFlagSweepCanon;
     int dead = -1;
     if (MIBN_SWEEP_DEAD_TAIL && canon && k == 5 && kout == 4) {
@@ -786,7 +878,13 @@
         for (int d = 0; d < 5; ++d)
             if (surv == packs[d]) dead = d;
     }
-    if (canon && k == 5 && kout == 5 && surv == 0x43210u) sweep_tiles_dma<5, true>(L, T, stw, 5, 3, F, outp, Rcells, t_begin, t_end, kout, surv, tid, tb);
+    if (gwords) {
+        const uint32_t *gw = sh_step + uni(words);
+        if (kout == 5 && surv == 0x43210u) sweep_tiles_dma<5, true, false, false, true>(L, T, stw, 5, 3, F, outp, Rcells, t_begin, t_end, kout, surv, tid, tb, -1, gw);
+        else if (dead >= 0) sweep_tiles_dma<5, true, true, false, true>(L, T, stw, 5, 3, F, outp, Rcells, t_begin, t_end, kout, surv, tid, tb, dead, gw);
+        else sweep_tiles_dma<5, false, false, false, true>(L, T, stw, 5, 3, F, outp, Rcells, t_begin, t_end, kout, surv, tid, tb, -1, gw);
+    }
+    else if (canon && k == 5 && kout == 5 && surv == 0x43210u) sweep_tiles_dma<5, true>(L, T, stw, 5, 3, F, outp, Rcells, t_begin, t_end, kout, surv, tid, tb);
     else if (dead >= 0) sweep_tiles_dma<5, true, true>(L, T, stw, 5, 3, F, outp, Rcells, t_begin, t_end, kout, surv, tid, tb, dead);
     else if (canon && k == 5) sweep_tiles_dma<5, false>(L, T, stw, 5, 3, F, outp, Rcells, t_begin, t_end, kout, surv, tid, tb);
     else if (canon && k == 4 && kout == 4 && surv == 0x3210u) sweep_tiles_dma<4, true>(L, T, stw, 4, 5, F, outp, Rcells, t_begin, t_end, kout, surv, tid, tb);
@@ -839,7 +937,9 @@
     double *__restrict__ slot = A.arena + A.arena_off[it.req];
     const uint32_t *p = A.prog + A.prog_off[it.req] + it.rel_off;
     const int words = (int)p[6];
-    for (int i = tid; i < words; i += kSweepWG) sh_step[i] = p[i];
+    const int gwords = uni((int)((it.a & kItemGrowFuse) ? (it.a >> kItemGrowWordsShift) & 0xffff : 0u));
+    const int it_tiles = (int)(it.a & kItemTilesMask);
+    for (int i = tid; i < words + gwords; i += kSweepWG) sh_step[i] = i < words ? p[i] : (p - gwords)[i - words];
     __syncthreads();
     const int k = uni((int)((sh_step[0] >> 16) & 0xff)), rb = uni((int)((sh_step[0] >> 24) & 0xff));
     const int tiles = uni((int)sh_step[3]);
@@ -851,10 +951,11 @@
     const double *__restrict__ F = slot + ((uint64_t)sh_step[kHdrWords] | ((uint64_t)sh_step[kHdrWords + 1] << 32));
     double *__restrict__ outp = slot + ((uint64_t)sh_step[4] | ((uint64_t)sh_step[5] << 32));
     const SweepTables tb{T, stw, smw, A.pool, slot, k, t_total};
-    const int t_begin = (int)((wg - it.b) * it.a);
-    const int t_end = min(tiles, t_begin + (int)it.a);
+    const int t_begin = (int)(wg - it.b) * it_tiles;
+    const int t_end = min(tiles, t_begin + it_tiles);
     const bool canon = (sh_step[1] >> 16) & kFlagSweepCanon;
-    if (canon && k == 5) sweep_tiles<5>(L, T, stw, F, outp, Rcells, t_begin, t_end, kout, surv, tid, tb);
+    if (gwords) sweep_tiles_impl<5, true>(L, T, stw, 5, 3, F, outp, Rcells, t_begin, t_end, kout, surv, tid, tb, sh_step + uni(words));
+    else if (canon && k == 5) sweep_tiles<5>(L, T, stw, F, outp, Rcells, t_begin, t_end, kout, surv, tid, tb);
     else if (canon && k == 4) sweep_tiles<4>(L, T, stw, F, outp, Rcells, t_begin, t_end, kout, surv, tid, tb);
     else if (canon && k == 3) sweep_tiles<3>(L, T, stw, F, outp, Rcells, t_begin, t_end, kout, surv, tid, tb);
     else sweep_tiles_any(L, T, stw, k, rb, F, outp, Rcells, t_begin, t_end, kout, surv, tid, tb);
```

New measurement: 297,300. 7.3% lower.
